# merijn-23/magr-ray-tracer

Hardware: AMD Instinct MI355X
Metric: Mrays/sec + extend-kernel HBM GB/s, sponza 1080p 256spp (higher is better)
Workload: dtype f32

## Files before the change

### include/rt355.h

```cpp
#ifndef RT355_H
#define RT355_H
#include "rt355_types.h"

#ifdef __cplusplus
extern "C" {
#endif

#define RT_OK            0
#define RT_E_INVALID    (-1)
#define RT_E_DEVICE     (-2)
#define RT_E_NOMEM      (-3)
#define RT_E_UNSUPPORTED (-4)

#define RT_SHADING_SIMPLE       0
#define RT_SHADING_NEE          1
#define RT_SAMPLING_HEMISPHERE  0
#define RT_SAMPLING_COSINE      1
#define RT_ACCEL_BVH2           0
#define RT_ACCEL_BVH4           1

typedef struct RtCtx RtCtx;

typedef struct RtConfig {
    int32_t width, height;
    int32_t y0, y1;
    int32_t max_bounces;
    int32_t shading, sampling, accel;
    int32_t russian_roulette;
    int32_t filter_fireflies;
    int32_t device;
    int32_t extend_variant;
    int32_t profile;
    int32_t shade_blocks_per_cu;
    int32_t persist_blocks_per_cu;
    int32_t builtins;
} RtConfig;

#define RT_BUILTINS_DEFAULT    0
#define RT_BUILTINS_IEEE       1
#define RT_BUILTINS_REFERENCE  2

typedef struct RtCounters {
    uint64_t extend_rays, extend_tlas_visits, extend_inst_visits, extend_node_visits, extend_prim_tests;
    uint64_t connect_rays, connect_tlas_visits, connect_inst_visits, connect_node_visits, connect_prim_tests;
    uint64_t primary_rays;
    uint64_t shadow_rays;
    uint64_t frames;
    uint64_t extend_node_issues, extend_leaf_issues, connect_node_issues, connect_leaf_issues;
    uint64_t extend_loop_node_events, extend_loop_leaf_events, connect_loop_node_events, connect_loop_leaf_events;
} RtCounters;

typedef struct RtStageTimes {
    double  generate_ms, extend_ms, shade_ms, compact_ms, connect_ms, accumulate_ms;
    int64_t generate_launches, extend_launches, shade_launches, compact_launches, connect_launches, accumulate_launches;
} RtStageTimes;

typedef struct RtKernelInfo {
    int32_t layout;
    int32_t persist, persist4;
    int32_t stack_entries;
    int32_t persist_grid, persist_grid_connect, shade_grid;
    int32_t n_blas;
} RtKernelInfo;

const char* rt_last_error(void);
int rt_device_count(void);
int rt_kernel_info(RtCtx* ctx, RtKernelInfo* out);
int rt_builtins(RtCtx* ctx);
int rt_top_levels(RtCtx* ctx, int32_t* extend, int32_t* connect);
typedef struct RtTraversalFacts {
    int32_t accel, extend_variant, persist_blocks_per_cu;
    int32_t layout;
    int32_t singleBlas;
    int32_t tlasDepth;
    int32_t nInterior, nQuads;
    int32_t stackEntries;
    int32_t sharedMemPerBlock;
    int32_t xcdFirst;
} RtTraversalFacts;
#define RT_TUNE_FIELDS 11
typedef struct RtTraversalPlan {
    int32_t trav;
    int32_t spillCap;
    int32_t coherent;
    int32_t topAuto;
    int32_t tuneBlocks, connectBlocks;
    int32_t tune[RT_TUNE_FIELDS], tuneConnect[RT_TUNE_FIELDS], tune4[RT_TUNE_FIELDS];
} RtTraversalPlan;
int rt_debug_traversal_plan(const RtTraversalFacts* facts, RtTraversalPlan* out);
int rt_debug_traversal_facts(RtCtx* ctx, RtTraversalFacts* out);
int rt_shade_footprint(RtCtx* ctx, int32_t* ldsBytes, int32_t* traversalBeside);
int rt_shade_tables(RtCtx* ctx, int32_t* capacityRows, int32_t* staged);

int rt_create(const RtConfig* cfg, RtCtx** out);
int rt_destroy(RtCtx* ctx);

int rt_upload_scene(RtCtx* ctx,
                    const RtPrimitive* prims, int32_t nPrims,
                    const RtMaterial* mats, int32_t nMats,
                    const RtFloat4* textures, int32_t nTexels,
                    const uint32_t* lights, int32_t nLights,
                    const void* bvhNodes, int32_t nNodes,
                    const uint32_t* primIdx, int32_t nIdx,
                    const RtTLASNode* tlas, int32_t nTlas,
                    const RtBVHInstance* blas, int32_t nBlas);

int rt_upload_scene_bvh2(RtCtx* ctx,
                         const RtPrimitive* prims, int32_t nPrims, const RtMaterial* mats, int32_t nMats,
                         const RtFloat4* textures, int32_t nTexels, const uint32_t* lights, int32_t nLights,
                         const RtBVHNode2* bvhNodes, int32_t nNodes, const uint32_t* primIdx, int32_t nIdx,
                         const RtTLASNode* tlas, int32_t nTlas, const RtBVHInstance* blas, int32_t nBlas);

int rt_validate_scene(int32_t accel,
                      const RtPrimitive* prims, int32_t nPrims, const RtMaterial* mats, int32_t nMats,
                      const RtFloat4* textures, int32_t nTexels, const uint32_t* lights, int32_t nLights,
                      const void* bvhNodes, int32_t nNodes, const uint32_t* primIdx, int32_t nIdx,
                      const RtTLASNode* tlas, int32_t nTlas, const RtBVHInstance* blas, int32_t nBlas);

int rt_share_scene(RtCtx* ctx, RtCtx* from);

int rt_build_bvh2(int32_t device, const RtBuildOptions* opts, const RtPrimitive* prims, int32_t nPrims, int32_t first, int32_t count,
                  uint32_t nodeBase, uint32_t idxBase, RtBVHNode2* nodes, int32_t nodeCap, int32_t* nNodes, uint32_t* primIdx,
                  RtBuildStats* stats);
int rt_build_bvh2_sah(int32_t device, const RtPrimitive* prims, int32_t nPrims, int32_t first, int32_t count, uint32_t nodeBase,
                      uint32_t idxBase, RtBVHNode2* nodes, int32_t nodeCap, int32_t* nNodes, uint32_t* primIdx, RtBuildStats* stats);
int rt_debug_sah_phases(float* out);
int rt_build_bvh2_sbvh(int32_t device, float alpha, const RtPrimitive* prims, int32_t nPrims, int32_t first, int32_t count,
                       uint32_t nodeBase, uint32_t idxBase, RtBVHNode2* nodes, int32_t nodeCap, int32_t* nNodes, uint32_t* primIdx,
                       int32_t idxCap, int32_t* nIdx, RtSbvhStats* stats);
int rt_debug_sbvh_phases(float* out);
int rt_build_bvh4(int32_t device, const RtBVHNode2* nodes2, int32_t nNodes, int32_t nIdx, const uint32_t* roots, int32_t nRoots,
                  RtBVHNode4* out4, RtBvh4Stats* stats);

typedef struct RtUpdateStats {
    double  gpu_ms;
    int32_t prims, nodes;
    int32_t tlas_nodes, tlas_depth;
    int32_t reconfigured;
    int32_t reserved[3];
} RtUpdateStats;
int rt_update_scene(RtCtx* ctx, const RtPrimitive* prims, int32_t first, int32_t count, const RtBVHInstance* blas, int32_t nBlas,
                    RtUpdateStats* stats);
#define RT_REBUILD_SAH   0
#define RT_REBUILD_LBVH  1
#define RT_REBUILD_SBVH  2
#define RT_REBUILD_REFIT 3
typedef struct RtRebuildStats {
    double  gpu_ms;
    double  wall_ms;
    double  stage_ms, build_ms, derive_ms, tlas_ms, commit_ms;
    int32_t prims, blas_built;
    int32_t nodes, n_idx;
    int32_t max_depth;
    int32_t tlas_nodes, tlas_depth;
    int32_t reconfigured;
    int32_t spatial_splits, prims_clipped;
} RtRebuildStats;
int rt_rebuild_scene(RtCtx* ctx, const RtPrimitive* prims, int32_t first, int32_t count, const RtBVHInstance* blas, int32_t nBlas,
                     int32_t builder, const RtBuildOptions* opts, RtRebuildStats* stats);
#define RT_REBUILD_KEEP  4
#define RT_REBUILD_REFIT_RANGE 5
int rt_rebuild_ranges(RtCtx* ctx, const RtPrimitive* prims, int32_t first, int32_t count, const RtBVHInstance* blas, int32_t nBlas,
                      const int32_t* plan, int32_t nRanges,
                      const RtBuildOptions* opts, RtRebuildStats* stats);
int rt_scene_blas_blocks(RtCtx* ctx, int32_t* n, int32_t* primFirst, int32_t* primCount, int32_t* nodes, int32_t* idxSlots, int32_t* compact, int32_t cap);
int rt_rebuild_ranges_check(int32_t nPrims, const int32_t* rangeFirst, const int32_t* rangeCount, const int32_t* compact, int32_t nBound,
                            const int32_t* plan, int32_t nRanges, int32_t first, int32_t count, const RtBuildOptions* opts);
typedef struct RtSceneShape {
    int32_t nRanges;
    const int32_t* rangeCount;
    int32_t nBlas;
    const int32_t* instRange;
    const RtBVHInstance* blas;
} RtSceneShape;
int rt_resize_scene(RtCtx* ctx, const void* prims, int32_t nPrims, const RtSceneShape* shape, int32_t builder, const RtBuildOptions* opts,
// ... 178 lines not shown
```

### magr_ray_tracer_amd/_lib.py

```python
import ctypes as C
import os

import numpy as np

_PKG = os.path.dirname(os.path.abspath(__file__))

f4 = np.dtype((np.float32, 4))
Ray = np.dtype([("O", f4), ("D", f4), ("rD", f4), ("N", f4), ("I", f4), ("intensity", f4), ("t", "<f4"),
                ("primIdx", "<i4"), ("bounces", "<i4"), ("pixelIdx", "<i4"), ("inside", "u1"), ("lastSpecular", "u1"),
                ("_pad0", "u1", 2), ("u", "<f4"), ("v", "<f4"), ("_pad1", "<u4")], align=False)
ShadowRay = np.dtype([("I", f4), ("L", f4), ("Nl", f4), ("intensity", f4), ("BRDF", f4), ("lightIdx", "<i4"),
                      ("pixelIdx", "<i4"), ("dotNL", "<f4"), ("dist", "<f4")])
Material = np.dtype([("color", f4), ("absorption", f4), ("specular", "<f4"), ("n1", "<f4"), ("n2", "<f4"),
                     ("isDielectric", "u1"), ("_pad0", "u1", 3), ("texIdx", "<i4"), ("texW", "<i4"), ("texH", "<i4"),
                     ("isLight", "u1"), ("_pad1", "u1", 3), ("emittance", f4)])
Primitive = np.dtype([("v0", f4), ("v1", f4), ("v2", f4), ("N", f4), ("centroid", f4), ("uv0", "<f4", 2), ("uv1", "<f4", 2),
                      ("uv2", "<f4", 2), ("_padt", "<f4", 2), ("objType", "<i4"), ("matIdx", "<i4"), ("area", "<f4"),
                      ("_pad", "<u4")])
Camera = np.dtype([("type", "<i4"), ("fov", "<f4"), ("aperture", "<f4"), ("focalLength", "<f4"), ("forward", f4),
                   ("right", f4), ("up", f4), ("origin", f4), ("horizontal", f4), ("vertical", f4), ("topLeft", f4)])
Settings = np.dtype([("numPrimitives", "<i4"), ("numLights", "<i4"), ("tracerType", "<i4"), ("frames", "<i4"),
                     ("antiAliasing", "<i4"), ("numInRays", "<i4"), ("numOutRays", "<i4"), ("shadowRays", "<i4"),
                     ("renderBVH", "<i4"), ("focalLength", "<f4")])
BVHNode2 = np.dtype([("aabbMin", f4), ("aabbMax", f4), ("first", "<u4"), ("count", "<u4"), ("_pad", "<u4", 2)])
# ... 20 lines not shown
SbvhStats = np.dtype([(n, "<i4") for n in ("nodes", "leaves", "n_idx", "depth", "spatial_splits", "prims_clipped", "forced_leaves", "levels")] +
                     [("sah_cost", "<f4"), ("device_ms", "<f4"), ("wall_ms", "<f4"), ("peak_refs", "<i4")])
Bvh4Stats = np.dtype([(n, "<i4") for n in ("live_nodes", "levels", "stack_need", "largest_leaf")] + [("device_ms", "<f4"), ("wall_ms", "<f4")])
Hit = np.dtype([("t", "<f4"), ("primIdx", "<i4"), ("u", "<f4"), ("v", "<f4")])
RayBatch = np.dtype([("origin", "<u8"), ("dir", "<u8"), ("originStride", "<i8"), ("dirStride", "<i8"), ("tmax", "<u8"), ("n", "<i8")])
TraceOut = np.dtype([("hit", "<u8"), ("point", "<u8"), ("normal", "<u8"), ("occluded", "<u8")])
TRACE_CLOSEST, TRACE_ANY = 0, 1
REALLYFAR = np.float32(1e30)
KernelInfo = np.dtype([(n, "<i4") for n in ("layout", "persist", "persist4", "stack_entries", "persist_grid", "persist_grid_connect",
                                             "shade_grid", "n_blas")])
TUNE_FIELDS = ("chunk", "refill", "inner", "leafK", "fixedChunks", "flat", "xcdRays", "xcdFirst", "thin", "topLevels", "topBase")
TraversalFacts = np.dtype([(n, "<i4") for n in ("accel", "extend_variant", "persist_blocks_per_cu", "layout", "singleBlas", "tlasDepth", "nInterior",
                                                 "nQuads", "stackEntries", "sharedMemPerBlock", "xcdFirst")])
TraversalPlan = np.dtype([(n, "<i4") for n in ("trav", "spillCap", "coherent", "topAuto", "tuneBlocks", "connectBlocks")] +
                         [(n, "<i4", len(TUNE_FIELDS)) for n in ("tune", "tuneConnect", "tune4")])
TRAV_NESTED, TRAV_BVH2, TRAV_TLAS, TRAV_TLAS_SPILL, TRAV_BVH4, TRAV_BVH4_TLAS, TRAV_BVH4_TLAS_SPILL = range(7)
assert TraversalFacts.itemsize == 44 and TraversalPlan.itemsize == 156

_SIZES = {"Ray": (Ray, 128), "ShadowRay": (ShadowRay, 96), "Material": (Material, 80), "Primitive": (Primitive, 128),
          "Camera": (Camera, 128), "Settings": (Settings, 40), "BVHNode2": (BVHNode2, 48), "BVHNode4": (BVHNode4, 160),
          "BVHInstance": (BVHInstance, 68), "TLASNode": (TLASNode, 48), "BuildOptions": (BuildOptions, 16), "BuildStats": (BuildStats, 32), "SbvhStats": (SbvhStats, 48), "Bvh4Stats": (Bvh4Stats, 24), "ShadowRecord": (ShadowRecord, 48), "Config": (Config, 64),
          "Hit": (Hit, 16), "RayBatch": (RayBatch, 48), "TraceOut": (TraceOut, 32)}
for _n, (_d, _s) in _SIZES.items():
    assert _d.itemsize == _s, (_n, _d.itemsize, _s)

SHADING_SIMPLE, SHADING_NEE = 0, 1
SAMPLING_HEMISPHERE, SAMPLING_COSINE = 0, 1
ACCEL_BVH2, ACCEL_BVH4 = 0, 1
PRIM_SPHERE, PRIM_PLANE, PRIM_TRIANGLE = 0, 1, 2
MATH_EXP, MATH_SIN, MATH_COS, MATH_ACOS, MATH_ATAN, MATH_F2I, MATH_ATAN2, MATH_SPHERE_TEXEL, MATH_NORMALIZE4, MATH_LENGTH4 = range(10)
MATH_WORDS = {MATH_EXP: (1, 1), MATH_SIN: (1, 1), MATH_COS: (1, 1), MATH_ACOS: (1, 1), MATH_ATAN: (1, 1), MATH_F2I: (1, 1),
              MATH_ATAN2: (2, 1), MATH_SPHERE_TEXEL: (6, 2), MATH_NORMALIZE4: (4, 4), MATH_LENGTH4: (4, 1)}
MATH_SWEEP_BLOCK_BITS = 20
MAX_BOUNCES = 7
BUILTINS_DEFAULT, BUILTINS_IEEE, BUILTINS_REFERENCE = 0, 1, 2
BUILTINS = {None: BUILTINS_DEFAULT, "ieee": BUILTINS_IEEE, "reference": BUILTINS_REFERENCE}


def builtins_value(name):
    try:
        return BUILTINS[name]
    except (KeyError, TypeError):
        raise ValueError(f"builtins must be None, 'ieee' or 'reference', not {name!r}") from None


RT_OK, RT_E_INVALID, RT_E_DEVICE, RT_E_NOMEM, RT_E_UNSUPPORTED = 0, -1, -2, -3, -4
SCENE_ARRAYS = {"prims": 0, "bvh": 1, "tlas": 2, "instances": 3, "pairs": 4, "triRecs": 5, "shadeRecs": 6, "lightRecs": 7,
                "tlasPairs": 8, "tlasPairsP": 9, "instRecs": 10}
SCENE_ARRAYS_BVH4 = {"quads": 11, "rootEntry": 12, "bvh2Kept": 13}
SCENE_ARRAYS_RESIZE = {"lights": 14}
SCENE_ARRAYS_MATERIALS = {"materials": 15, "textures": 16}
MaterialUpdate = np.dtype([("mats", "<u8"), ("nMats", "<i4"), ("_pad0", "<i4"), ("texels", "<u8"), ("texFirst", "<i4"), ("texCount", "<i4"),
                           ("nTexels", "<i4"), ("_pad1", "<i4"), ("primMat", "<u8"), ("primFirst", "<i4"), ("primCount", "<i4")])
assert MaterialUpdate.itemsize == 56
MaterialStats = np.dtype([("gpu_ms", "<f8"), ("wall_ms", "<f8")] +
                         [(n, "<i4") for n in ("mats", "texels", "prims", "lights", "tables_staged_changed", "atlas_reallocated")] +
                         [("reserved", "<i4", 2)])
assert MaterialStats.itemsize == 48
SceneShape = np.dtype([("nRanges", "<i4"), ("_pad0", "<i4"), ("rangeCount", "<u8"), ("nBlas", "<i4"), ("_pad1", "<i4"), ("instRange", "<u8"),
                       ("blas", "<u8")])
assert SceneShape.itemsize == 40
Geometry = np.dtype([("first", "<i4"), ("count", "<i4"), ("prims", "<u8"), ("positions", "<u8"), ("positionStride", "<i8"), ("nVertices", "<i8"),
                     ("indices", "<u8")])
assert Geometry.itemsize == 48
UpdateStats = np.dtype([("gpu_ms", "<f8"), ("prims", "<i4"), ("nodes", "<i4"), ("tlas_nodes", "<i4"), ("tlas_depth", "<i4"),
                        ("reconfigured", "<i4"), ("reserved", "<i4", 3)])
assert UpdateStats.itemsize == 40
REBUILD_SAH, REBUILD_LBVH, REBUILD_SBVH = 0, 1, 2
REBUILD_REFIT = 3
REBUILD_KEEP = 4
REBUILD_REFIT_RANGE = 5
RANGES_INFO_FIELDS = ("built", "kept", "refit", "pairs_derived", "pairs_relocated", "slots_derived", "slots_relocated", "nodes_numbered", "leaves_refit")
RangesInfo = np.dtype([(n, "<i4") for n in RANGES_INFO_FIELDS] + [("reserved", "<i4", 3)])
assert RangesInfo.itemsize == 48
RefitInfo = np.dtype([(n, "<i4") for n in ("path", "live_quads", "changed_nodes", "stack_need")])
assert RefitInfo.itemsize == 16
REFIT_NONE, REFIT_IN_PLACE, REFIT_RECOLLAPSED, REFIT_FORCED = 0, 1, 2, 3
RebuildStats = np.dtype([(n, "<f8") for n in ("gpu_ms", "wall_ms", "stage_ms", "build_ms", "derive_ms", "tlas_ms", "commit_ms")] +
                        [(n, "<i4") for n in ("prims", "blas_built", "nodes", "n_idx", "max_depth", "tlas_nodes", "tlas_depth", "reconfigured")] +
                        [("spatial_splits", "<i4"), ("prims_clipped", "<i4")])
assert RebuildStats.itemsize == 96

DEVICE_SYMBOLS = [
    "rt_last_error", "rt_device_count", "rt_kernel_info", "rt_builtins", "rt_top_levels", "rt_shade_footprint", "rt_shade_tables", "rt_create", "rt_destroy", "rt_upload_scene", "rt_share_scene", "rt_set_seeds", "rt_seed_default",
    "rt_get_seeds", "rt_bind_accum", "rt_accum_device_ptr", "rt_stream", "rt_reset", "rt_render", "rt_synchronize", "rt_focus",
    "rt_read_accum", "rt_write_accum", "rt_postproc", "rt_read_counters", "rt_reset_counters", "rt_read_stage_times", "rt_reset_stage_times", "rt_set_profile",
    "rt_stage_begin_frame", "rt_stage_generate", "rt_stage_extend", "rt_stage_shade", "rt_stage_connect",
    "rt_debug_get_rays", "rt_debug_set_rays", "rt_debug_get_shadow", "rt_debug_enable_steps", "rt_debug_get_steps", "rt_debug_math",
    "rt_debug_math_sweep", "rt_debug_math_mode", "rt_debug_math_sweep_mode", "rt_validate_scene", "rt_build_bvh2", "rt_build_bvh2_sah", "rt_debug_sah_phases", "rt_build_bvh2_sbvh", "rt_debug_sbvh_phases", "rt_update_scene", "rt_group_update_scene", "rt_debug_get_scene_array",
    "rt_rebuild_scene", "rt_group_rebuild_scene", "rt_blas_ranges", "rt_debug_rebuild_allocations", "rt_refit_info",
    "rt_build_bvh4", "rt_upload_scene_bvh2", "rt_group_upload_scene_bvh2",
    "rt_group_create", "rt_group_destroy", "rt_group_lanes", "rt_group_concurrency", "rt_group_stream_class", "rt_group_class_concurrency", "rt_group_lane", "rt_group_frames", "rt_group_upload_scene", "rt_group_share_scene",
    "rt_group_seed", "rt_group_reset", "rt_group_render", "rt_group_synchronize", "rt_group_sum", "rt_group_read_accum", "rt_group_focus",
    "rt_group_postproc", "rt_trace", "rt_trace_window", "rt_resize_scene", "rt_group_resize_scene", "rt_resize_check",
    "rt_update_materials", "rt_group_update_materials", "rt_materials_check",
    "rt_rebuild_ranges", "rt_group_rebuild_ranges", "rt_scene_blas_blocks", "rt_rebuild_ranges_check", "rt_blas_blocks",
    "rt_debug_traversal_plan", "rt_debug_traversal_facts", "rt_ranges_info", "rt_debug_derive_pairs", "rt_debug_relocate_pairs",
    "rt_update_geometry", "rt_rebuild_geometry", "rt_rebuild_geometry_ranges", "rt_group_update_geometry", "rt_group_rebuild_geometry",
    "rt_group_rebuild_geometry_ranges", "rt_geometry_check"]
HOST_SYMBOLS = [
    "rth_last_error", "rth_scene_create", "rth_scene_destroy", "rth_add_material", "rth_add_texture", "rth_load_texture", "rth_add_sphere",
    "rth_add_plane", "rth_add_triangle", "rth_add_quad", "rth_add_triangles", "rth_build_blas", "rth_build_bvh4",
    "rth_build_tlas", "rth_bvh4_from_nodes", "rth_set_instance_transform", "rth_primitives", "rth_materials", "rth_textures", "rth_lights",
    "rth_bvh2_nodes", "rth_bvh4_nodes", "rth_prim_idx", "rth_tlas_nodes", "rth_blas_nodes", "rth_bvh_stats", "rth_camera",
    "rth_renderer_create", "rth_renderer_destroy", "rth_renderer_init", "rth_renderer_set_camera", "rth_renderer_tick",
    "rth_renderer_read", "rth_renderer_camera", "rth_seed_stream", "rth_load_model", "rth_save_png",
    "rth_set_build_threads", "rth_renderer_save_frame", "rth_renderer_camera_move", "rth_renderer_camera_mouse", "rth_renderer_camera_zoom", "rth_renderer_frames", "rth_renderer_set_lanes", "rth_renderer_set_builtins", "rth_renderer_builtins",
    "rth_build_blas_lbvh", "rth_build_bvh2_lbvh", "rth_lbvh_stats", "rth_set_primitives", "rth_refit",
    "rth_build_blas_sah_gpu", "rth_build_bvh2_sah", "rth_build_blas_sbvh_gpu", "rth_build_bvh2_sbvh", "rth_rebuild", "rth_blas_ranges",
    "rth_build_bvh4_gpu", "rth_build_bvh4_levels", "rth_bvh4_refit", "rth_refit_bvh4", "rth_add_instance", "rth_light_list",
    "rth_set_materials", "rth_set_texels", "rth_set_prim_materials", "rth_rebuild_ranges", "rth_swap_instances", "rth_set_vertices"]

_dev = None
_host = None


class NativeLibraryMissing(RuntimeError):
    pass


def _load(name, local=False):
    path = os.path.join(_PKG, name)
    if not os.path.exists(path):
        raise NativeLibraryMissing(
            f"{path} is missing: build it with `python -m magr_ray_tracer_amd.build` (hipcc, gfx950). "
            "The hot path has no Python/CPU fallback.")
    return C.CDLL(path, mode=C.RTLD_LOCAL if local else C.RTLD_GLOBAL)


_variants = {}


def device_lib(variant=None):
    global _dev
    if variant:
        if variant not in _variants:
            keep, _dev = _dev, None
            try:
                _variants[variant] = _bind_device(_load(f"librt355_{variant}.so", local=True))
            finally:
                _dev = keep
        return _variants[variant]
    if _dev is None:
        _dev = _bind_device(_load("librt355.so"))
    return _dev


def _bind_device(lib):
    if True:
        vp, i32, i64 = C.c_void_p, C.c_int32, C.c_int64
        lib.rt_last_error.restype = C.c_char_p
        lib.rt_create.argtypes = [vp, C.POINTER(vp)]
        lib.rt_kernel_info.argtypes = [vp, vp]
        lib.rt_builtins.argtypes = [vp]
        lib.rt_top_levels.argtypes = [vp, C.POINTER(i32), C.POINTER(i32)]
        lib.rt_debug_traversal_plan.argtypes = [vp, vp]
        lib.rt_debug_traversal_facts.argtypes = [vp, vp]
        lib.rt_shade_footprint.argtypes = [vp, C.POINTER(i32), C.POINTER(i32)]
        lib.rt_shade_tables.argtypes = [vp, C.POINTER(i32), C.POINTER(i32)]
        lib.rt_destroy.argtypes = [vp]
        lib.rt_upload_scene.argtypes = [vp, vp, i32, vp, i32, vp, i32, vp, i32, vp, i32, vp, i32, vp, i32, vp, i32]
        lib.rt_upload_scene_bvh2.argtypes = lib.rt_upload_scene.argtypes
        lib.rt_group_upload_scene_bvh2.argtypes = lib.rt_upload_scene.argtypes
        lib.rt_build_bvh4.argtypes = [i32, vp, i32, i32, vp, i32, vp, vp]
        lib.rt_share_scene.argtypes = [vp, vp]
        lib.rt_set_seeds.argtypes = [vp, vp, i64]
        lib.rt_seed_default.argtypes = [vp]
        lib.rt_get_seeds.argtypes = [vp, vp, i64]
        lib.rt_bind_accum.argtypes = [vp, vp]
        lib.rt_accum_device_ptr.argtypes = [vp]
        lib.rt_accum_device_ptr.restype = vp
        lib.rt_stream.argtypes = [vp]
        lib.rt_stream.restype = vp
        lib.rt_reset.argtypes = [vp]
        lib.rt_render.argtypes = [vp, vp, vp, i32]
        lib.rt_synchronize.argtypes = [vp]
        lib.rt_focus.argtypes = [vp, i32, i32, vp, C.POINTER(C.c_float)]
        lib.rt_read_accum.argtypes = [vp, vp]
        lib.rt_read_counters.argtypes = [vp, vp]
        lib.rt_write_accum.argtypes = [vp, vp]
        lib.rt_postproc.argtypes = [vp, i32, C.c_float, C.c_float, C.c_float, vp, vp]
        lib.rt_reset_counters.argtypes = [vp]
        lib.rt_read_stage_times.argtypes = [vp, vp]
        lib.rt_reset_stage_times.argtypes = [vp]
        lib.rt_set_profile.argtypes = [vp, i32]
        lib.rt_stage_begin_frame.argtypes = [vp]
        lib.rt_stage_generate.argtypes = [vp, vp, vp]
        lib.rt_stage_extend.argtypes = [vp, i32, i32]
        lib.rt_stage_shade.argtypes = [vp, i32]
        lib.rt_stage_connect.argtypes = [vp, i32, i32]
        lib.rt_debug_get_rays.argtypes = [vp, i32, vp, i32, C.POINTER(i32)]
        lib.rt_debug_set_rays.argtypes = [vp, i32, vp, i32]
        lib.rt_trace.argtypes = [vp, i32, vp, vp]
        lib.rt_trace_window.argtypes = [vp]
        lib.rt_trace_window.restype = i64
        lib.rt_debug_get_shadow.argtypes = [vp, i32, i32, vp, i32, C.POINTER(i32)]
        lib.rt_debug_get_steps.argtypes = [vp, vp, i32, C.POINTER(i32)]
        lib.rt_debug_enable_steps.argtypes = [vp, i32]
        lib.rt_debug_math.argtypes = [i32, vp, vp, i64]
        lib.rt_debug_math_sweep.argtypes = [i32, i32, i32, vp]
        lib.rt_debug_math_mode.argtypes = [i32, i32, vp, vp, i64]
        lib.rt_debug_math_sweep_mode.argtypes = [i32, i32, i32, i32, vp]
        lib.rt_validate_scene.argtypes = [i32, vp, i32, vp, i32, vp, i32, vp, i32, vp, i32, vp, i32, vp, i32, vp, i32]
        lib.rt_build_bvh2.argtypes = [i32, vp, vp, i32, i32, i32, C.c_uint32, C.c_uint32, vp, i32, C.POINTER(i32), vp, vp]
        lib.rt_build_bvh2_sah.argtypes = [i32, vp, i32, i32, i32, C.c_uint32, C.c_uint32, vp, i32, C.POINTER(i32), vp, vp]
        lib.rt_debug_sah_phases.argtypes = [vp]
        lib.rt_build_bvh2_sbvh.argtypes = [i32, C.c_float, vp, i32, i32, i32, C.c_uint32, C.c_uint32, vp, i32, C.POINTER(i32), vp, i32, C.POINTER(i32), vp]
        lib.rt_debug_sbvh_phases.argtypes = [vp]
        lib.rt_update_scene.argtypes = [vp, vp, i32, i32, vp, i32, vp]
        lib.rt_group_update_scene.argtypes = [vp, vp, i32, i32, vp, i32, vp]
        lib.rt_debug_get_scene_array.argtypes = [vp, i32, vp, i64, C.POINTER(i64)]
        lib.rt_rebuild_scene.argtypes = [vp, vp, i32, i32, vp, i32, i32, vp, vp]
        lib.rt_group_rebuild_scene.argtypes = [vp, vp, i32, i32, vp, i32, i32, vp, vp]
        lib.rt_debug_rebuild_allocations.argtypes = [vp, vp]
        lib.rt_rebuild_ranges.argtypes = [vp, vp, i32, i32, vp, i32, vp, i32, vp, vp]
        lib.rt_group_rebuild_ranges.argtypes = [vp, vp, i32, i32, vp, i32, vp, i32, vp, vp]
        lib.rt_scene_blas_blocks.argtypes = [vp, vp, vp, vp, vp, vp, vp, i32]
        lib.rt_rebuild_ranges_check.argtypes = [i32, vp, vp, vp, i32, vp, i32, i32, i32, vp]
        lib.rt_blas_blocks.argtypes = [vp, i32, vp, i32, i32, vp, i32, vp, vp, vp, vp, vp, vp, i32]
        lib.rt_update_geometry.argtypes = [vp, vp, vp, i32, vp]
        lib.rt_group_update_geometry.argtypes = [vp, vp, vp, i32, vp]
        lib.rt_rebuild_geometry.argtypes = [vp, vp, vp, i32, i32, vp, vp]
        lib.rt_group_rebuild_geometry.argtypes = [vp, vp, vp, i32, i32, vp, vp]
        lib.rt_rebuild_geometry_ranges.argtypes = [vp, vp, vp, i32, vp, i32, vp, vp]
        lib.rt_group_rebuild_geometry_ranges.argtypes = [vp, vp, vp, i32, vp, i32, vp, vp]
        lib.rt_geometry_check.argtypes = [vp, i32, vp]
        lib.rt_resize_scene.argtypes = [vp, vp, i32, vp, i32, vp, vp]
        lib.rt_group_resize_scene.argtypes = [vp, vp, i32, vp, i32, vp, vp]
        lib.rt_resize_check.argtypes = [i32, vp, i32, vp]
        lib.rt_update_materials.argtypes = [vp, vp, vp]
        lib.rt_group_update_materials.argtypes = [vp, vp, vp]
        lib.rt_materials_check.argtypes = [vp, i32, i32]
        lib.rt_refit_info.argtypes = [vp, vp]
        lib.rt_ranges_info.argtypes = [vp, vp]
        lib.rt_debug_derive_pairs.argtypes = [vp, i32, vp, i32, vp, vp, i32, vp, C.POINTER(i32)]
        lib.rt_debug_relocate_pairs.argtypes = [vp, i32, C.c_uint32, C.c_uint32, vp]
        lib.rt_blas_ranges.argtypes = [vp, i32, vp, i32, i32, vp, i32, vp, vp]
        lib.rt_group_create.argtypes = [vp, i32, C.POINTER(vp)]
        lib.rt_group_destroy.argtypes = [vp]
        lib.rt_group_lanes.argtypes = [vp]
        lib.rt_group_concurrency.argtypes = [vp]
        lib.rt_group_stream_class.argtypes = [vp]
# ... 107 lines not shown
```

### magr_ray_tracer_amd/csrc/ctx.h

```cpp
#pragma once
#include <algorithm>
#include <memory>
#include <vector>
#include "rt355_dev.h"
#include "scene_dev.h"

struct RtCtx {
    RtConfig cfg{};
    hipStream_t stream = nullptr;
    hipStream_t home = nullptr;
    bool queued = true;
    rt355dev::DevScene sc{};
    rt355dev::DevQueues q{};
    rt355dev::DevVariant var{};
    int nPix = 0, firstPixel = 0, gridMax = 0;
    int cuCount = 0; size_t ldsPerBlock = 0, ldsPerCU = 0;
    bool sceneLoaded = false, ownAccum = true;
    std::shared_ptr<scenedev::SceneBag> scene;
    uint64_t sceneGen = 0;
    scenedev::SceneFacts facts;
    std::vector<void*> queueAllocs;
    float* dFocus = nullptr;
    RtRay* dRayIO = nullptr;
    uint64_t frames = 0, primaryRays = 0;
    struct Ev { hipEvent_t a, b; int stage; };
    std::vector<Ev> evPool; size_t evUsed = 0;
    RtStageTimes times{};
    int trav = 0;
    int coherent = 1;
    uint32_t* dSpill = nullptr; size_t spillWords = 0;
    int xcdFirst = -1;
    int spillCap = 0;
    bool cursorUsed[2 * (RT_MAX_BOUNCES + 2)] = {};
    bool shadeRun[RT_MAX_BOUNCES + 1] = {};
    bool generated = false;
    int persistGrid = 0, persistGridConnect = 0;
    rt355dev::PersistTune tune{}, tuneConnect{}, tune4{};
    int tuneBlocks = 0, connectBlocks = 0;
    float4* dPostF = nullptr; uchar4* dPostB = nullptr;
    int32_t* dSteps = nullptr;
    struct TraceView { rt355dev::DevQueues q{}; bool ready = false; std::vector<void*> words; float4* rays[3] = {}; size_t cap = 0; } tv;
    int shadeTile = rt355dev::kTile;
    int shadeGrid = 1024;
    void (*kGenerate)(rt355dev::DevQueues, RtCamera, int, int) = nullptr;
    void (*kShade)(rt355dev::DevScene, rt355dev::DevQueues, rt355dev::DevVariant, int) = nullptr;
    void (*kFocus)(rt355dev::DevScene, RtCamera, int, int, int, int, float*) = nullptr;
};

static inline dim3 grid_for(int n) { return dim3((unsigned)std::max(1, (n + rt355dev::kBlock - 1) / rt355dev::kBlock)); }
__attribute__((visibility("hidden"))) void ctx_free(RtCtx* ctx);
__attribute__((visibility("hidden"))) int postproc(RtCtx* ctx, const float4* accum, int32_t frames, float vignette, float gamma, float chromatic,
                                                    RtFloat4* outF32, uint8_t* outRGBA8);
```

### magr_ray_tracer_amd/csrc/rt355.hip

```cpp
#include <hip/hip_runtime.h>
#include <hip/hip_ext.h>
#include <algorithm>
#include <cstdio>
#include <cmath>
#include <cstdlib>
#include <cstring>
#include <memory>
#include <atomic>
#include <string>
#include <vector>
#include "../../include/rt355.h"
#include "rt355_kernels.h"
#include "ctx.h"
#include "geometry_common.h"

using namespace rt355dev;
using namespace scenedev;

static_assert(kColumnLanes == kBlock && kTopLevelsMax == kTopMaxLevels && sizeof(float4) * 4 == 64, "trav_common.h computes with the kernels' sizes");
static thread_local std::string g_err;
int rt355_set_error(int code, const char* msg) { g_err = msg; return code; }

template <bool REFB> static void choose_builtin_kernels_of(RtCtx* ctx)
{
    const bool nee = ctx->cfg.shading == RT_SHADING_NEE, small = ctx->shadeTile == 256;
    ctx->kGenerate = k_generate<REFB>;
    ctx->kShade = nee ? (small ? k_shade<true, 256, REFB> : k_shade<true, kTile, REFB>) : (small ? k_shade<false, 256, REFB> : k_shade<false, kTile, REFB>);
    ctx->kFocus = ctx->cfg.accel == RT_ACCEL_BVH4 ? k_focus<RT_ACCEL_BVH4, REFB> : k_focus<RT_ACCEL_BVH2, REFB>;
}
static void choose_builtin_kernels(RtCtx* ctx)
{
    if (ctx->cfg.builtins == RT_BUILTINS_REFERENCE) choose_builtin_kernels_of<true>(ctx);
    else choose_builtin_kernels_of<false>(ctx);
}
enum { ST_GENERATE, ST_EXTEND, ST_SHADE, ST_COMPACT, ST_CONNECT, ST_ACCUM };

extern "C" const char* rt_last_error(void) { return g_err.c_str(); }
extern "C" int rt_device_count(void) { int n = 0; if (hipGetDeviceCount(&n) != hipSuccess) return 0; return n; }
static int sync_scene_config(RtCtx* ctx);
extern "C" int rt_builtins(RtCtx* ctx)
{
    if (!ctx) return fail(RT_E_INVALID, "rt_builtins: null context");
    return ctx->cfg.builtins;
}
extern "C" int rt_kernel_info(RtCtx* ctx, RtKernelInfo* out)
{
    if (!ctx || !out) return fail(RT_E_INVALID, "rt_kernel_info: null argument");
    if (!ctx->sceneLoaded) return fail(RT_E_INVALID, "rt_kernel_info: no scene uploaded");
    if (const int rc = sync_scene_config(ctx)) return rc;
    const int persist = ctx->trav <= TRAV_TLAS_SPILL ? ctx->trav : 0;
    const int persist4 = ctx->trav == TRAV_BVH4 ? 1 : (ctx->trav == TRAV_BVH4_TLAS ? 2 : (ctx->trav == TRAV_BVH4_TLAS_SPILL ? 3 : 0));
    *out = RtKernelInfo{ ctx->facts.layout, persist, persist4, spill_trav(ctx->trav) ? ctx->spillCap : ctx->facts.stackEntries, ctx->persistGrid, ctx->persistGridConnect,
                         ctx->shadeGrid, ctx->sc.nBlas };
    return RT_OK;
}

extern "C" int rt_top_levels(RtCtx* ctx, int32_t* extend, int32_t* connect)
{
    if (!ctx || !extend || !connect) return fail(RT_E_INVALID, "rt_top_levels: null argument");
    if (!ctx->sceneLoaded) return fail(RT_E_INVALID, "rt_top_levels: no scene uploaded");
    if (const int rc = sync_scene_config(ctx)) return rc;
    *extend = ctx->tune.topLevels; *connect = ctx->tuneConnect.topLevels;
    return RT_OK;
}

static int beside_shade(const RtCtx* c, int stage, int topLevels, int* perCU, int* shadeLds);
extern "C" int rt_shade_footprint(RtCtx* ctx, int32_t* ldsBytes, int32_t* traversalBeside)
{
    if (!ctx || !ldsBytes || !traversalBeside) return fail(RT_E_INVALID, "rt_shade_footprint: null argument");
    if (!ctx->sceneLoaded) return fail(RT_E_INVALID, "rt_shade_footprint: no scene uploaded");
    if (const int rc = sync_scene_config(ctx)) return rc;
    *ldsBytes = 0; *traversalBeside = 0;
    if (!persistent(ctx->trav)) {
        hipFuncAttributes a{};
        HIPCHK(hipFuncGetAttributes(&a, (const void*)ctx->kShade));
        *ldsBytes = (int32_t)a.sharedSizeBytes;
        return RT_OK;
    }
    int lds = 0, beside = 0;
    if (const int rc = beside_shade(ctx, ST_EXTEND, 0, &beside, &lds)) return rc;
    *ldsBytes = lds; *traversalBeside = beside;
    return RT_OK;
}

extern "C" int rt_shade_tables(RtCtx* ctx, int32_t* capacityRows, int32_t* staged)
{
    if (!ctx || !capacityRows || !staged) return fail(RT_E_INVALID, "rt_shade_tables: null argument");
    if (!ctx->sceneLoaded) return fail(RT_E_INVALID, "rt_shade_tables: no scene uploaded");
    if (const int rc = sync_scene_config(ctx)) return rc;
    *capacityRows = kShadeTableRows;
    *staged = ctx->var.shadeTables != 0 && shade_tables_fit(ctx->sc.nLights, ctx->sc.nMats);
    return RT_OK;
}

static void free_bag(std::vector<void*>& bag) { for (void* p : bag) (void)hipFree(p); bag.clear(); }

static void scene_release(RtCtx* ctx)
{
    if (!ctx->scene) return;
    auto& h = ctx->scene->holders;
    h.erase(std::remove(h.begin(), h.end(), ctx), h.end());
    ctx->scene.reset();
}
static void scene_hold(RtCtx* ctx, const std::shared_ptr<SceneBag>& bag)
{
    scene_release(ctx);
    ctx->scene = bag;
    bag->holders.push_back(ctx);
}
int SceneBag::wait_holders() const
{
    for (const RtCtx* h : holders) {
        HIPCHK(hipStreamSynchronize(h->stream));
        if (h->home != h->stream) HIPCHK(hipStreamSynchronize(h->home));
    }
    return RT_OK;
}

static int tlas_lds_entries(const RtCtx* c) { return tlas_lds_entries(c->trav, c->spillCap, c->facts.stackEntries, c->facts.tlasDepth); }
static size_t tlas_stack_bytes(const RtCtx* c) { return tlas_column_bytes(tlas_lds_entries(c)); }

using PersistKernel = void (*)(DevScene, DevQueues, int, int, int, PersistTune);
using NestedKernel = void (*)(DevScene, DevQueues, int, int);
struct TraceLaunch {
    PersistKernel persist = nullptr;
    NestedKernel nested = nullptr;
    dim3 grid;
    size_t lds = 0;
    PersistTune tune{};
};
static TraceLaunch trace_launch(const RtCtx* c, int stage, int bounce, bool steps, int rays, int topLevels = -1 )
{
    TraceLaunch L;
    L.grid = grid_for(rays);
    L.lds = stack_bytes(c->facts.stackEntries);
    const bool connect = stage == ST_CONNECT;
    const bool bvh4 = c->cfg.accel == RT_ACCEL_BVH4, l1 = c->facts.layout == 1;
    bool top = false;
    switch (c->trav) {
    case TRAV_NESTED:
        if (connect) L.nested = bvh4 ? (l1 ? k_connect<RT_ACCEL_BVH4, 1> : k_connect<RT_ACCEL_BVH4, 0>) : (l1 ? k_connect<RT_ACCEL_BVH2, 1> : k_connect<RT_ACCEL_BVH2, 0>);
        else L.nested = bvh4 ? (l1 ? k_extend<RT_ACCEL_BVH4, 1> : k_extend<RT_ACCEL_BVH4, 0>) : (l1 ? k_extend<RT_ACCEL_BVH2, 1> : k_extend<RT_ACCEL_BVH2, 0>);
        break;
    case TRAV_BVH2:
        L.tune = connect ? c->tuneConnect : c->tune;
        if (topLevels >= 0) L.tune.topLevels = topLevels;
        if (connect) { top = L.tune.topLevels > 0; L.persist = top ? k_trace_persist<true, false, false, true> : k_trace_persist<true>; L.grid = dim3(c->persistGridConnect); }
        else if (bounce > 0 || c->cfg.extend_variant == 3) {
            top = L.tune.topLevels > 0;
            if (top) L.persist = steps ? k_trace_persist<false, false, true, true> : k_trace_persist<false, false, false, true>;
            else L.persist = steps ? k_trace_persist<false, false, true> : k_trace_persist<false>;
            L.grid = dim3(c->persistGrid);
        }
        else if (c->cfg.extend_variant == 5) L.nested = k_extend<RT_ACCEL_BVH2, 1>;
        else L.persist = c->coherent ? k_trace_persist<false, true> : (steps ? k_trace_persist<false, false, true> : k_trace_persist<false>);
        if (top) { L.tune.topBase = c->facts.stackEntries * kBlock; L.lds += top_bytes(L.tune.topLevels); }
        break;
    case TRAV_BVH4:
        L.tune = connect ? c->tuneConnect : c->tune4;
        L.persist = connect ? k_trace_persist4<true> : k_trace_persist4<false>;
        if (connect || bounce > 0) L.grid = dim3(connect ? c->persistGridConnect : c->persistGrid);
        break;
    case TRAV_TLAS:
    case TRAV_TLAS_SPILL: {
        const bool spill = c->trav == TRAV_TLAS_SPILL;
        L.lds = tlas_stack_bytes(c);
        if (connect) {
            L.tune = c->tuneConnect;
            L.persist = spill ? k_trace_persist_tlas<true, false, true> : k_trace_persist_tlas<true>;
            L.grid = dim3(c->persistGridConnect);
            break;
        }
        L.tune = c->tune;
        if (bounce > 0 || spill) L.grid = dim3(c->persistGrid);
        const bool coh = c->coherent && (bounce == 0 || c->coherent == 2) && (c->tune.flat || !spill);
        if (steps) L.persist = spill ? k_trace_persist_tlas<false, true, true> : k_trace_persist_tlas<false, true>;
        else if (coh) L.persist = spill ? k_trace_persist_tlas<false, false, true, true> : k_trace_persist_tlas<false, false, false, true>;
        else L.persist = spill ? k_trace_persist_tlas<false, false, true> : k_trace_persist_tlas<false>;
        break;
    }
    case TRAV_BVH4_TLAS:
    case TRAV_BVH4_TLAS_SPILL: {
        const bool spill = c->trav == TRAV_BVH4_TLAS_SPILL;
        L.lds = tlas_stack_bytes(c);
        if (connect) {
            L.tune = c->tuneConnect;
            L.persist = spill ? k_trace_persist4_tlas<true, false, true> : k_trace_persist4_tlas<true>;
            L.grid = dim3(c->persistGridConnect);
            break;
        }
        L.tune = c->tune4;
        if (bounce > 0 || spill) L.grid = dim3(c->persistGrid);
        if (steps) L.persist = spill ? k_trace_persist4_tlas<false, true, true> : k_trace_persist4_tlas<false, true>;
        else L.persist = spill ? k_trace_persist4_tlas<false, false, true> : k_trace_persist4_tlas<false>;
        break;
    }
    }
    return L;
}

static int persist_query(const RtCtx* c, int stage, int topLevels, int* perCU)
{
    const TraceLaunch L = trace_launch(c, stage, stage == ST_CONNECT ? 0 : 1, false, c->nPix, topLevels);
    HIPCHK(hipOccupancyMaxActiveBlocksPerMultiprocessor(perCU, L.persist, kBlock, L.lds));
    return RT_OK;
}
static int persist_blocks(const RtCtx* c, int stage, int perCU)
{
    const bool connect = stage == ST_CONNECT;
    const int fit = std::max(1, perCU);
    int g = std::max(1, std::min(perCU, connect ? kAdmitAnySgpr : kAdmit96Sgpr));
    if (c->cfg.persist_blocks_per_cu > 0) g = std::min(g, std::min(c->cfg.persist_blocks_per_cu, fit));
    if (c->tuneBlocks > 0) g = std::min(c->tuneBlocks, fit);
    if (connect && c->connectBlocks > 0) g = std::min(c->connectBlocks, fit);
    return g;
}

static constexpr size_t kLdsBlock = 1280;
static int beside_shade(const RtCtx* c, int stage, int topLevels, int* perCU, int* shadeLds)
{
    const TraceLaunch L = trace_launch(c, stage, stage == ST_CONNECT ? 0 : 1, false, c->nPix, topLevels);
    hipFuncAttributes shade{}, trav{};
    HIPCHK(hipFuncGetAttributes(&shade, (const void*)c->kShade));
    HIPCHK(hipFuncGetAttributes(&trav, (const void*)L.persist));
    auto alloc = [](int regs) { return std::max(8, (regs + 7) / 8 * 8); };
    const size_t ldsCU = std::max(c->ldsPerCU, c->ldsPerBlock);
    auto blocks = [](size_t bytes) { return (bytes + kLdsBlock - 1) / kLdsBlock * kLdsBlock; };
    const size_t travLds = blocks(trav.sharedSizeBytes + L.lds), shadeLdsCU = blocks(shade.sharedSizeBytes);
    const int shadeWaves = std::max(1, c->shadeTile / kBlock);
    const int byLds = ldsCU > shadeLdsCU && travLds > 0 ? (int)((ldsCU - shadeLdsCU) / travLds) : 0;
    const int byVgpr = (512 - shadeWaves * alloc(shade.numRegs)) / alloc(trav.numRegs);
    const int bySlots = 8 - shadeWaves;
    *perCU = std::max(0, std::min(std::min(byLds, byVgpr), std::min(bySlots, stage == ST_CONNECT ? kAdmitAnySgpr : kAdmit96Sgpr)));
    *shadeLds = (int)shade.sharedSizeBytes;
    return RT_OK;
}

static constexpr size_t kEvRing = 4096;
static void ev_account(RtCtx* c, RtCtx::Ev& e)
{
    float ms = 0;
    if (hipEventElapsedTime(&ms, e.a, e.b) != hipSuccess) { (void)hipEventSynchronize(e.b); (void)hipEventElapsedTime(&ms, e.a, e.b); }
    switch (e.stage) {
    case ST_GENERATE: c->times.generate_ms += ms; c->times.generate_launches++; break;
// ... 84 lines not shown
        choose_builtin_kernels(ctx);
        HIPCHK(hipOccupancyMaxActiveBlocksPerMultiprocessor(&perCU, ctx->kShade, ctx->shadeTile, 0));
        perCU = std::min(perCU, kAdmitAnySgpr);
        ctx->shadeGrid = ctx->cuCount * std::max(1, perCU);
        if (c.shade_blocks_per_cu > 0 && c.shade_blocks_per_cu <= 16) ctx->shadeGrid = ctx->cuCount * c.shade_blocks_per_cu;
        if (knobs.perCU) ctx->shadeGrid = ctx->cuCount * knobs.perCU;
    }
    hipError_t e = hipStreamCreateWithFlags(&ctx->home, hipStreamNonBlocking);
    if (e != hipSuccess) return fail(RT_E_DEVICE, "hipStreamCreate failed: %s", hipGetErrorString(e));
    ctx->stream = ctx->home;
    DevQueues& q = ctx->q;
    const size_t n = (size_t)ctx->nPix, nS = n * (size_t)c.max_bounces;
    int rc = RT_OK;
    auto& bag = ctx->queueAllocs;
#define QA(field, count) if (rc == RT_OK) rc = dalloc(bag, &q.field, count)
    const size_t nTiles = (n + kBlock - 1) / kBlock;
    for (int k = 0; k < 2; k++) { QA(O[k], n); QA(D[k], n); QA(inten[k], n); QA(meta[k], n); QA(tile[k], nTiles + 2); QA(super[k], nTiles / 64 + 2); QA(supAcc[k], nTiles / 64 + 2); }
    QA(hit, n);
    QA(sA, nS); QA(sB, nS); QA(sC, nS);
    QA(nRays, RT_MAX_BOUNCES + 2); QA(nShadow, RT_MAX_BOUNCES + 2); QA(cursor, kCursorWords); QA(shadeTicket, (size_t)(RT_MAX_BOUNCES + 1) * kTicketClasses * kTicketStride); QA(fault, 1);
    QA(seeds, n); QA(accum, (size_t)c.width * c.height);
    if (rc == RT_OK) rc = dalloc(bag, &ctx->dSteps, n);
    q.steps = nullptr;
    QA(ctrExtend, (size_t)ctx->gridMax * kCtrCols); QA(ctrConnect, (size_t)ctx->gridMax * kCtrCols);
#undef QA
    if (rc == RT_OK) rc = dalloc(bag, &ctx->dFocus, 1);
    if (rc != RT_OK) return rc;
    q.nPix = ctx->nPix; q.firstPixel = ctx->firstPixel; q.width = c.width; q.height = c.height;
    (void)hipMemsetAsync(q.accum, 0, sizeof(float4) * (size_t)c.width * c.height, ctx->stream);
    (void)hipMemsetAsync(q.nRays, 0, sizeof(int32_t) * (RT_MAX_BOUNCES + 2), ctx->stream);
    (void)hipMemsetAsync(q.nShadow, 0, sizeof(int32_t) * (RT_MAX_BOUNCES + 2), ctx->stream);
    (void)hipMemsetAsync(q.cursor, 0, sizeof(int32_t) * kCursorWords, ctx->stream);
    (void)hipMemsetAsync(q.shadeTicket, 0, sizeof(int32_t) * (size_t)(RT_MAX_BOUNCES + 1) * kTicketClasses * kTicketStride, ctx->stream);
    (void)hipMemsetAsync(q.fault, 0, sizeof(int32_t), ctx->stream);
    (void)hipMemsetAsync(q.ctrExtend, 0, sizeof(unsigned long long) * (size_t)ctx->gridMax * kCtrCols, ctx->stream);
    (void)hipMemsetAsync(q.ctrConnect, 0, sizeof(unsigned long long) * (size_t)ctx->gridMax * kCtrCols, ctx->stream);
    for (int k = 0; k < 2; k++) {
        (void)hipMemsetAsync(q.tile[k], 0, sizeof(unsigned long long) * (nTiles + 2), ctx->stream);
        (void)hipMemsetAsync(q.super[k], 0, sizeof(unsigned long long) * (nTiles / 64 + 2), ctx->stream);
        (void)hipMemsetAsync(q.supAcc[k], 0, sizeof(unsigned long long) * (nTiles / 64 + 2), ctx->stream);
    }
    (void)hipMemsetAsync(q.hit, 0, sizeof(float4) * n, ctx->stream);
    HIPCHK(hipStreamSynchronize(ctx->stream));
    rc = rt_seed_default(ctx);
    if (rc != RT_OK) return rc;
    ev_init(ctx);
    *out = guard.release();
    return RT_OK;
}

void ctx_free(RtCtx* ctx)
{
    if (!ctx) return;
    (void)hipSetDevice(ctx->cfg.device);
    if (ctx->stream) (void)hipStreamSynchronize(ctx->stream);
    scene_release(ctx); free_bag(ctx->queueAllocs);
    if (ctx->dRayIO) (void)hipFree(ctx->dRayIO);
    free_bag(ctx->tv.words);
    for (float4* p : ctx->tv.rays) if (p) (void)hipFree(p);
    if (ctx->dSpill) (void)hipFree(ctx->dSpill);
    if (ctx->dPostF) (void)hipFree(ctx->dPostF);
    if (ctx->dPostB) (void)hipFree(ctx->dPostB);
    for (auto& e : ctx->evPool) { if (e.a) (void)hipEventDestroy(e.a); if (e.b) (void)hipEventDestroy(e.b); }
    if (ctx->home) (void)hipStreamDestroy(ctx->home);
    delete ctx;
}
extern "C" int rt_destroy(RtCtx* ctx)
{
    ctx_free(ctx);
    return RT_OK;
}

static TravFacts traversal_facts(const RtCtx* ctx)
{
    const SceneFacts& s = ctx->facts;
    return TravFacts{ ctx->cfg.accel, ctx->cfg.extend_variant, ctx->cfg.persist_blocks_per_cu, s.layout, s.singleBlas, s.tlasDepth, s.nInterior, s.nQuads, s.stackEntries,
                      (int)ctx->ldsPerBlock, ctx->xcdFirst };
}
static void adopt_plan(RtCtx* ctx, const TravPlan& p)
{
    ctx->trav = p.trav; ctx->spillCap = p.spillCap; ctx->coherent = p.coherent;
    ctx->tune = p.tune; ctx->tuneConnect = p.tuneConnect; ctx->tune4 = p.tune4;
    ctx->tuneBlocks = p.tuneBlocks; ctx->connectBlocks = p.connectBlocks;
}
static int fit_top_tables(RtCtx* ctx, bool topAuto)
{
    for (PersistTune* t : { &ctx->tune, &ctx->tuneConnect }) if (stack_bytes(ctx->facts.stackEntries) + top_bytes(t->topLevels) > ctx->ldsPerBlock) t->topLevels = 0;
    if (topAuto) for (int stage : { ST_EXTEND, ST_CONNECT }) {
        PersistTune& t = stage == ST_CONNECT ? ctx->tuneConnect : ctx->tune;
        int q = 0, lv = t.topLevels, beside = 0, shadeLds = 0;
        const bool shared = ctx->cfg.persist_blocks_per_cu > 0;
        if (const int rc = persist_query(ctx, stage, 0, &q)) return rc;
        const int base = persist_blocks(ctx, stage, q);
        if (shared) { if (const int rc = beside_shade(ctx, stage, 0, &beside, &shadeLds)) return rc; }
        for (; lv > 0; lv--) {
            if (const int rc = persist_query(ctx, stage, lv, &q)) return rc;
            if (persist_blocks(ctx, stage, q) != base) continue;
            if (!shared) break;
            int fit = 0;
            if (const int rc = beside_shade(ctx, stage, lv, &fit, &shadeLds)) return rc;
            if (fit >= beside) break;
        }
        t.topLevels = lv;
    }
    return RT_OK;
}
static int size_persistent_grids(RtCtx* ctx)
{
    int perCU = 0;
    if (const int rc = persist_query(ctx, ST_EXTEND, -1, &perCU)) return rc;
    int perCUc = perCU;
    if (bvh4_tlas_trav(ctx->trav) || ctx->tuneConnect.topLevels > 0) { if (const int rc = persist_query(ctx, ST_CONNECT, -1, &perCUc)) return rc; }
    ctx->persistGrid = std::min(ctx->gridMax, persist_blocks(ctx, ST_EXTEND, perCU) * ctx->cuCount);
    ctx->persistGridConnect = std::min(ctx->gridMax, persist_blocks(ctx, ST_CONNECT, perCUc) * ctx->cuCount);
    return RT_OK;
}
static int bind_spill_columns(RtCtx* ctx)
{
    ctx->q.spill = nullptr; ctx->q.spillStride = 0; ctx->q.stackCap = 0;
    ctx->q.tlasLdsEntries = tlas_trav(ctx->trav) ? (uint32_t)tlas_lds_entries(ctx) : 0u;
    if (!spill_trav(ctx->trav)) return RT_OK;
    const size_t stride = (size_t)std::max(ctx->persistGrid, ctx->persistGridConnect) * kBlock;
    const size_t words = stride * (size_t)(tlas_stack_entries(ctx->facts.stackEntries, ctx->facts.tlasDepth) - ctx->spillCap);
    if (words > ctx->spillWords) {
        if (ctx->dSpill) (void)hipFree(ctx->dSpill);
        ctx->dSpill = nullptr; ctx->spillWords = 0;
        if (hipMalloc((void**)&ctx->dSpill, words * sizeof(uint32_t)) != hipSuccess) return fail(RT_E_NOMEM, "hipMalloc of the spill stacks (%zu bytes) failed", words * sizeof(uint32_t));
        ctx->spillWords = words;
    }
    ctx->q.spill = ctx->dSpill; ctx->q.spillStride = (uint32_t)stride; ctx->q.stackCap = (uint32_t)ctx->spillCap;
    return RT_OK;
}
static int configure_traversal(RtCtx* ctx)
{
    static std::atomic<int> serial{ 0 };
    if (ctx->xcdFirst < 0) ctx->xcdFirst = serial.fetch_add(1) & 7;
    const TravPlan plan = plan_traversal(traversal_facts(ctx), read_trav_knobs());
    adopt_plan(ctx, plan);
    if (persistent(ctx->trav)) {
        if (const int rc = fit_top_tables(ctx, plan.topAuto)) return rc;
        if (const int rc = size_persistent_grids(ctx)) return rc;
    } else ctx->persistGrid = ctx->persistGridConnect = 0;
    return bind_spill_columns(ctx);
}

static void frame_state_reset(RtCtx* ctx);
static int adopt_scene(RtCtx* ctx)
{
    const SceneBag& b = *ctx->scene;
    const SceneArrays& a = b.sc;
    if (ctx->sceneLoaded && ctx->sc.nPrims != a.nPrims) {
        const DevQueues& q = ctx->q;
        HIPCHK(hipMemsetAsync(q.nRays, 0, sizeof(int32_t) * (RT_MAX_BOUNCES + 2), ctx->stream));
        HIPCHK(hipMemsetAsync(q.nShadow, 0, sizeof(int32_t) * (RT_MAX_BOUNCES + 2), ctx->stream));
        HIPCHK(hipMemsetAsync(q.cursor, 0, sizeof(int32_t) * kCursorWords, ctx->stream));
        HIPCHK(hipMemsetAsync(q.shadeTicket, 0, sizeof(int32_t) * (size_t)(RT_MAX_BOUNCES + 1) * kTicketClasses * kTicketStride, ctx->stream));
        HIPCHK(hipMemsetAsync(q.hit, 0, sizeof(float4) * (size_t)ctx->nPix, ctx->stream));
        ctx->queued = true;
        frame_state_reset(ctx);
    }
    auto f4 = [](const RtFloat4* p) { return (const float4*)p; };
    ctx->sc = DevScene{ a.prims, a.mats, f4(a.tex), a.lights, a.bvh2, a.bvh4, a.primIdx, a.tlas, a.blas, f4(a.pairs), f4(a.triRecs), a.rootEntry, f4(a.shadeRecs),
                        f4(a.tlasPairs), f4(a.instRecs), a.tlasRoot, f4(a.tlasPairsP), a.tlasRootP, f4(a.lightRecs), f4(a.quads), a.nLights, a.nPrims, a.nBlas, a.nTex, a.nMats };
    ctx->facts = b.facts;
    const int rc = configure_traversal(ctx);
    if (rc == RT_OK) ctx->sceneGen = b.generation;
// ... 272 lines not shown
    return RT_OK;
}
extern "C" int rt_bind_accum(RtCtx* ctx, void* devicePtr)
{
    if (!ctx) return fail(RT_E_INVALID, "rt_bind_accum: null context");
    HIPCHK(hipSetDevice(ctx->cfg.device));
    HIPCHK(hipStreamSynchronize(ctx->stream));
    if (devicePtr) { ctx->q.accum = (float4*)devicePtr; ctx->ownAccum = false; }
    else if (!ctx->ownAccum) {
        float4* a = nullptr;
        int rc = dalloc(ctx->queueAllocs, &a, (size_t)ctx->cfg.width * ctx->cfg.height);
        if (rc != RT_OK) return rc;
        HIPCHK(hipMemset(a, 0, sizeof(float4) * (size_t)ctx->cfg.width * ctx->cfg.height));
        ctx->q.accum = a; ctx->ownAccum = true;
    }
    return RT_OK;
}
extern "C" void* rt_accum_device_ptr(RtCtx* ctx) { return ctx ? (void*)ctx->q.accum : nullptr; }
extern "C" void* rt_stream(RtCtx* ctx) { if (ctx) ctx->queued = true; return ctx ? (void*)ctx->stream : nullptr; }

extern "C" int rt_reset(RtCtx* ctx)
{
    if (!ctx) return fail(RT_E_INVALID, "rt_reset: null context");
    HIPCHK(hipSetDevice(ctx->cfg.device));
    ctx->queued = true;
    hipLaunchKernelGGL(k_reset, dim3((ctx->nPix + kBlock - 1) / kBlock), dim3(kBlock), 0, ctx->stream, ctx->q.accum, ctx->firstPixel, ctx->nPix);
    HIPCHK(hipGetLastError());
    return RT_OK;
}

static int need_scene(RtCtx* ctx, const char* who)
{
    if (!ctx) return fail(RT_E_INVALID, "%s: null context", who);
    if (!ctx->sceneLoaded) return fail(RT_E_INVALID, "%s: no scene uploaded", who);
    return sync_scene_config(ctx);
}

static void frame_state_reset(RtCtx* ctx)
{
    memset(ctx->cursorUsed, 0, sizeof ctx->cursorUsed);
    memset(ctx->shadeRun, 0, sizeof ctx->shadeRun);
    ctx->generated = false;
}
extern "C" int rt_stage_begin_frame(RtCtx* ctx)
{
    if (!ctx) return fail(RT_E_INVALID, "rt_stage_begin_frame: null context");
    ctx->queued = true;
    hipLaunchKernelGGL(k_begin_frame, dim3(1), dim3(256), 0, ctx->stream, ctx->q);
    HIPCHK(hipGetLastError());
    frame_state_reset(ctx);
    return RT_OK;
}
static int generate(RtCtx* ctx, const RtCamera* cam, const RtSettings* s, int beginFrame)
{
    if (beginFrame) frame_state_reset(ctx);
    ctx->queued = true;
    LAUNCH(ctx, ST_GENERATE, ctx->kGenerate, grid_for(ctx->nPix), 0, ctx->q, *cam, s ? s->antiAliasing : 1, beginFrame);
    HIPCHK(hipGetLastError());
    ctx->primaryRays += (uint64_t)ctx->nPix;
    ctx->generated = true;
    return RT_OK;
}
extern "C" int rt_stage_generate(RtCtx* ctx, const RtCamera* cam, const RtSettings* s)
{
    if (!ctx || !cam) return fail(RT_E_INVALID, "rt_stage_generate: null argument");
    return generate(ctx, cam, s, 0);
}
extern "C" int rt_stage_extend(RtCtx* ctx, int32_t bounce, int32_t renderBVH)
{
    int rc = need_scene(ctx, "rt_stage_extend"); if (rc) return rc;
    ctx->queued = true;
    if (bounce < 0 || bounce > ctx->cfg.max_bounces) return fail(RT_E_INVALID, "rt_stage_extend: bounce %d outside [0, %d]", bounce, ctx->cfg.max_bounces);
    if (persistent(ctx->trav)) {
        if (ctx->cursorUsed[bounce]) HIPCHK(hipMemsetAsync(ctx->q.cursor + bounce, 0, sizeof(int32_t), ctx->stream));
        ctx->cursorUsed[bounce] = true;
    }
    const bool wantSteps = renderBVH != 0 || ctx->q.steps != nullptr;
    const TraceLaunch L = trace_launch(ctx, ST_EXTEND, bounce, wantSteps, ctx->nPix);
    if (L.persist) LAUNCH(ctx, ST_EXTEND, L.persist, L.grid, L.lds, ctx->sc, ctx->q, bounce, bounce, renderBVH, L.tune);
    else LAUNCH(ctx, ST_EXTEND, L.nested, L.grid, L.lds, ctx->sc, ctx->q, bounce, renderBVH);
    HIPCHK(hipGetLastError());
    return RT_OK;
}
extern "C" int rt_stage_shade(RtCtx* ctx, int32_t bounce)
{
    int rc = need_scene(ctx, "rt_stage_shade"); if (rc) return rc;
    ctx->queued = true;
    if (bounce < 0 || bounce >= ctx->cfg.max_bounces) return fail(RT_E_INVALID, "rt_stage_shade: bounce %d outside [0, %d)", bounce, ctx->cfg.max_bounces);
    if (ctx->shadeRun[bounce] || (bounce > 0 && !ctx->shadeRun[bounce - 1]) || (bounce == 0 && !ctx->generated)) {
        const size_t nTiles = ((size_t)ctx->nPix + kBlock - 1) / kBlock;
        HIPCHK(hipMemsetAsync(ctx->q.tile[bounce & 1], 0, sizeof(unsigned long long) * (nTiles + 2), ctx->stream));
        HIPCHK(hipMemsetAsync(ctx->q.super[bounce & 1], 0, sizeof(unsigned long long) * (nTiles / 64 + 2), ctx->stream));
        HIPCHK(hipMemsetAsync(ctx->q.supAcc[bounce & 1], 0, sizeof(unsigned long long) * (nTiles / 64 + 2), ctx->stream));
        HIPCHK(hipMemsetAsync(ctx->q.shadeTicket + (size_t)bounce * kTicketClasses * kTicketStride, 0, sizeof(int32_t) * (size_t)kTicketClasses * kTicketStride, ctx->stream));
    }
    const int tileSz = ctx->shadeTile;
    const dim3 sg((unsigned)std::max(1, std::min(ctx->shadeGrid, (ctx->nPix + tileSz - 1) / tileSz)));
    LAUNCHB(ctx, ST_SHADE, ctx->kShade, sg, tileSz, 0, ctx->sc, ctx->q, ctx->var, bounce);
    ctx->shadeRun[bounce] = true;
    HIPCHK(hipGetLastError());
    return RT_OK;
}
extern "C" int rt_stage_connect(RtCtx* ctx, int32_t b0, int32_t b1)
{
    int rc = need_scene(ctx, "rt_stage_connect"); if (rc) return rc;
    ctx->queued = true;
    if (b0 < 0 || b1 < b0 || b1 >= ctx->cfg.max_bounces) return fail(RT_E_INVALID, "rt_stage_connect: bounce range [%d,%d] outside [0, %d)", b0, b1, ctx->cfg.max_bounces);
    if (persistent(ctx->trav)) {
        const int ci = (RT_MAX_BOUNCES + 2) + b0;
        if (ctx->cursorUsed[ci]) HIPCHK(hipMemsetAsync(ctx->q.cursor + ci, 0, sizeof(int32_t), ctx->stream));
        ctx->cursorUsed[ci] = true;
    }
    const TraceLaunch L = trace_launch(ctx, ST_CONNECT, b0, false, ctx->nPix * (b1 - b0 + 1));
    if (L.persist) LAUNCH(ctx, ST_CONNECT, L.persist, L.grid, L.lds, ctx->sc, ctx->q, b0, b1, 0, L.tune);
    else LAUNCH(ctx, ST_CONNECT, L.nested, L.grid, L.lds, ctx->sc, ctx->q, b0, b1);
    ev_begin(ctx, ST_ACCUM);
    for (int b = b0; b <= b1; b++)
        hipLaunchKernelGGL(k_accumulate, dim3(std::min(grid_for(ctx->nPix).x, 2048u)), dim3(kBlock), 0, ctx->stream, ctx->q, b);
    ev_end(ctx, ST_ACCUM);
    HIPCHK(hipGetLastError());
    return RT_OK;
}

static constexpr int64_t kTraceWindowMax = (int64_t)1 << 22;
static int64_t trace_window(const RtCtx* ctx)
{
    int64_t w = std::min<int64_t>((int64_t)ctx->gridMax * kBlock, kTraceWindowMax);
    if (const char* t = getenv("RT355_TRACE_WINDOW")) { const long long k = atoll(t); if (k > 0) w = std::min<int64_t>(w, k); }
    return w;
}
extern "C" int64_t rt_trace_window(RtCtx* ctx)
{
    if (!ctx) return fail(RT_E_INVALID, "rt_trace_window: null context");
    return trace_window(ctx);
}
static int device_pointer(const RtCtx* ctx, const char* who, const char* name, const void* p, int64_t bytes, int align, bool hostAllowed, bool* onDevice)
{
    if ((uintptr_t)p % (uintptr_t)align) return fail(RT_E_INVALID, "%s: %s (%p) is not aligned to %d bytes", who, name, p, align);
    hipPointerAttribute_t a{};
    const hipError_t e = hipPointerGetAttributes(&a, p);
    if (e != hipSuccess) (void)hipGetLastError();
    const bool device = e == hipSuccess && a.type == hipMemoryTypeDevice && a.device == ctx->cfg.device;
    const bool shared = e == hipSuccess && (a.type == hipMemoryTypeManaged || (a.type == hipMemoryTypeHost && a.devicePointer == p));
    const bool host = e != hipSuccess || a.type == hipMemoryTypeUnregistered || a.type == hipMemoryTypeHost;
    if (!device && !shared && !(hostAllowed && host))
        return fail(RT_E_INVALID, "%s: %s (%p) is not memory accessible from device %d (a host pointer? memory of another GPU?)", who, name, p, ctx->cfg.device);
    if (device) {
        hipDeviceptr_t base = nullptr; size_t size = 0;
        if (hipMemGetAddressRange(&base, &size, (hipDeviceptr_t)p) != hipSuccess) (void)hipGetLastError();
        else if ((const char*)p + bytes > (const char*)base + size)
            return fail(RT_E_INVALID, "%s: %s needs %lld bytes from %p, its allocation ends %lld bytes earlier", who, name, (long long)bytes, p,
                        (long long)(((const char*)p + bytes) - ((const char*)base + size)));
    }
    if (onDevice) *onDevice = device || shared;
    return RT_OK;
}
static int trace_pointer(const RtCtx* ctx, const char* name, const void* p, int64_t bytes, int align) { return device_pointer(ctx, "rt_trace", name, p, bytes, align, false); }
static int trace_view(RtCtx* ctx, size_t ownRays)
{
    RtCtx::TraceView& v = ctx->tv;
    if (!v.ready) {
        DevQueues q{};
        unsigned long long* ctr = nullptr;
        int rc = dalloc(v.words, &q.nRays, RT_MAX_BOUNCES + 2);
        if (rc == RT_OK) rc = dalloc(v.words, &q.nShadow, RT_MAX_BOUNCES + 2);
        if (rc == RT_OK) rc = dalloc(v.words, &q.cursor, kCursorWords);
        if (rc == RT_OK) rc = dalloc(v.words, &q.fault, 1);
        if (rc == RT_OK) rc = dalloc(v.words, &ctr, (size_t)ctx->gridMax * kCtrCols);
        if (rc != RT_OK) { free_bag(v.words); return rc; }
        HIPCHK(hipMemsetAsync(q.nRays, 0, sizeof(int32_t) * (RT_MAX_BOUNCES + 2), ctx->stream));
        HIPCHK(hipMemsetAsync(q.nShadow, 0, sizeof(int32_t) * (RT_MAX_BOUNCES + 2), ctx->stream));
        HIPCHK(hipMemsetAsync(q.cursor, 0, sizeof(int32_t) * kCursorWords, ctx->stream));
        HIPCHK(hipMemsetAsync(q.fault, 0, sizeof(int32_t), ctx->stream));
        HIPCHK(hipMemsetAsync(ctr, 0, sizeof(unsigned long long) * (size_t)ctx->gridMax * kCtrCols, ctx->stream));
        q.ctrExtend = q.ctrConnect = ctr;
        q.nPix = ctx->nPix; q.firstPixel = ctx->firstPixel; q.width = ctx->cfg.width; q.height = ctx->cfg.height;
        v.q = q; v.ready = true;
    }
    if (ownRays > v.cap) {
        HIPCHK(hipStreamSynchronize(ctx->stream));
        for (float4*& p : v.rays) { if (p) (void)hipFree(p); p = nullptr; }
        v.cap = 0;
        for (float4*& p : v.rays)
            if (hipMalloc((void**)&p, ownRays * sizeof(float4)) != hipSuccess) {
                (void)hipGetLastError();
                for (float4*& r : v.rays) { if (r) (void)hipFree(r); r = nullptr; }
                return fail(RT_E_NOMEM, "rt_trace: hipMalloc of the query's ray arrays (3 x %zu bytes) failed", ownRays * sizeof(float4));
            }
        v.cap = ownRays;
    }
    return RT_OK;
}
extern "C" int rt_trace(RtCtx* ctx, int32_t mode, const RtRayBatch* rays, const RtTraceOut* out)
{
    if (!ctx) return fail(RT_E_INVALID, "rt_trace: null ctx");
    if (!rays) return fail(RT_E_INVALID, "rt_trace: null rays");
    if (!out) return fail(RT_E_INVALID, "rt_trace: null out");
    int rc = need_scene(ctx, "rt_trace"); if (rc) return rc;
    if (mode != RT_TRACE_CLOSEST && mode != RT_TRACE_ANY) return fail(RT_E_INVALID, "rt_trace: mode %d is neither RT_TRACE_CLOSEST (0) nor RT_TRACE_ANY (1)", mode);
    const bool any = mode == RT_TRACE_ANY;
    const int64_t n = rays->n;
    if (n < 0) return fail(RT_E_INVALID, "rt_trace: rays->n = %lld is negative", (long long)n);
    if (rays->originStride < 12 || rays->originStride % 4) return fail(RT_E_INVALID, "rt_trace: rays->originStride = %lld must be >= 12 and a multiple of 4", (long long)rays->originStride);
    if (rays->dirStride < 12 || rays->dirStride % 4) return fail(RT_E_INVALID, "rt_trace: rays->dirStride = %lld must be >= 12 and a multiple of 4", (long long)rays->dirStride);
    if (any) {
        if (out->hit || out->point || out->normal) return fail(RT_E_INVALID, "rt_trace: out->%s is not produced by RT_TRACE_ANY", out->hit ? "hit" : (out->point ? "point" : "normal"));
    } else if (out->occluded) return fail(RT_E_INVALID, "rt_trace: out->occluded is not produced by RT_TRACE_CLOSEST");
    if (n == 0) return RT_OK;
    if (any ? !out->occluded : !out->hit) return fail(RT_E_INVALID, "rt_trace: out->%s is required by %s", any ? "occluded" : "hit", any ? "RT_TRACE_ANY" : "RT_TRACE_CLOSEST");
    if (!rays->origin) return fail(RT_E_INVALID, "rt_trace: null rays->origin");
    if (!rays->dir) return fail(RT_E_INVALID, "rt_trace: null rays->dir");
    HIPCHK(hipSetDevice(ctx->cfg.device));
    if ((rc = trace_pointer(ctx, "rays->origin", rays->origin, (n - 1) * rays->originStride + 12, 4))) return rc;
    if ((rc = trace_pointer(ctx, "rays->dir", rays->dir, (n - 1) * rays->dirStride + 12, 4))) return rc;
    if (rays->tmax) if ((rc = trace_pointer(ctx, "rays->tmax", rays->tmax, n * 4, 4))) return rc;
    if (out->hit) if ((rc = trace_pointer(ctx, "out->hit", out->hit, n * 16, 16))) return rc;
    if (out->point) if ((rc = trace_pointer(ctx, "out->point", out->point, n * 16, 16))) return rc;
    if (out->normal) if ((rc = trace_pointer(ctx, "out->normal", out->normal, n * 16, 16))) return rc;
    if (out->occluded) if ((rc = trace_pointer(ctx, "out->occluded", out->occluded, n, 1))) return rc;
    const bool vecO = rays->originStride == 16 && (uintptr_t)rays->origin % 16 == 0, vecD = rays->dirStride == 16 && (uintptr_t)rays->dir % 16 == 0;
    const bool inPlace = !any && vecO && vecD && !rays->tmax && !out->point && !out->normal;
    const int64_t window = trace_window(ctx);
    if ((rc = trace_view(ctx, inPlace ? 0 : (size_t)std::min(n, window)))) return rc;
    ctx->queued = true;
    DevQueues q = ctx->tv.q;
    q.spill = ctx->q.spill; q.spillStride = ctx->q.spillStride; q.stackCap = ctx->q.stackCap; q.tlasLdsEntries = ctx->q.tlasLdsEntries;
    for (int64_t off = 0; off < n; off += window) {
        const int m = (int)std::min(window, n - off);
        TraceIO io{ (const char*)rays->origin + off * rays->originStride, (const char*)rays->dir + off * rays->dirStride, rays->originStride, rays->dirStride,
                    rays->tmax ? rays->tmax + off : nullptr, out->hit ? (float4*)out->hit + off : nullptr, out->point ? (float4*)out->point + off : nullptr,
                    out->normal ? (float4*)out->normal + off : nullptr, out->occluded ? out->occluded + off : nullptr };
        float4* const* own = ctx->tv.rays;
        q.O[kTraceBounce & 1] = q.sA = inPlace ? (float4*)io.origin : own[0];
        q.D[kTraceBounce & 1] = q.sB = inPlace ? (float4*)io.dir : own[1];
        q.hit = q.sC = inPlace ? io.hit : own[2];
        hipLaunchKernelGGL(k_trace_arm, dim3(1), dim3(1), 0, ctx->stream, q, m, (int)any);
        if (!inPlace) hipLaunchKernelGGL(k_trace_load, grid_for(m), dim3(kBlock), 0, ctx->stream, q, io, m, (int)any, (int)vecO, (int)vecD);
        const TraceLaunch L = trace_launch(ctx, any ? ST_CONNECT : ST_EXTEND, kTraceBounce, false, m);
        if (L.persist) hipLaunchKernelGGL(L.persist, L.grid, dim3(kBlock), L.lds, ctx->stream, ctx->sc, q, kTraceBounce, kTraceBounce, 0, L.tune);
        else if (any) hipLaunchKernelGGL(L.nested, L.grid, dim3(kBlock), L.lds, ctx->stream, ctx->sc, q, kTraceBounce, kTraceBounce);
        else hipLaunchKernelGGL(L.nested, L.grid, dim3(kBlock), L.lds, ctx->stream, ctx->sc, q, kTraceBounce, 0);
        if (!inPlace) hipLaunchKernelGGL(k_trace_store, grid_for(m), dim3(kBlock), 0, ctx->stream, ctx->sc, q, io, m, (int)any);
        HIPCHK(hipGetLastError());
    }
    return RT_OK;
}

extern "C" int rt_render(RtCtx* ctx, const RtCamera* cam, const RtSettings* settings, int32_t frames)
{
    int rc = need_scene(ctx, "rt_render"); if (rc) return rc;
    if (!cam) return fail(RT_E_INVALID, "rt_render: null camera");
    if (frames <= 0) return fail(RT_E_INVALID, "rt_render: frames must be > 0");
    HIPCHK(hipSetDevice(ctx->cfg.device));
    const bool nee = ctx->cfg.shading == RT_SHADING_NEE, rr = ctx->cfg.russian_roulette != 0;
    const int renderBVH = settings ? settings->renderBVH : 0;
    for (int f = 0; f < frames; f++) {
        if ((rc = generate(ctx, cam, settings, 1))) return rc;
        for (int b = 0; b < ctx->cfg.max_bounces; b++) {
            if ((rc = rt_stage_extend(ctx, b, renderBVH))) return rc;
            if (renderBVH) break;
            if ((rc = rt_stage_shade(ctx, b))) return rc;
            if (!rr && nee) if ((rc = rt_stage_connect(ctx, b, b))) return rc;
        }
        if (rr && nee && !renderBVH) if ((rc = rt_stage_connect(ctx, 0, ctx->cfg.max_bounces - 1))) return rc;
        ctx->frames++;
    }
    return RT_OK;
}
static int check_fault(RtCtx* ctx)
{
    int32_t f = 0;
    HIPCHK(hipMemcpy(&f, ctx->q.fault, sizeof f, hipMemcpyDeviceToHost));
    if (f) {
        (void)hipMemset(ctx->q.fault, 0, sizeof f);
        return fail(RT_E_DEVICE, "device fault 0x%08x: a bounded wait of the ordered scan in k_shade expired (results of this render are invalid)", (unsigned)f);
    }
    return RT_OK;
}
extern "C" int rt_synchronize(RtCtx* ctx)
{
    if (!ctx) return fail(RT_E_INVALID, "rt_synchronize: null context");
    HIPCHK(hipSetDevice(ctx->cfg.device));
    HIPCHK(hipStreamSynchronize(ctx->stream));
    ev_collect(ctx);
    return check_fault(ctx);
}

extern "C" int rt_focus(RtCtx* ctx, int32_t x, int32_t y, const RtCamera* cam, float* t)
{
    int rc = need_scene(ctx, "rt_focus"); if (rc) return rc;
    if (!cam || !t) return fail(RT_E_INVALID, "rt_focus: null argument");
    HIPCHK(hipSetDevice(ctx->cfg.device));
    hipLaunchKernelGGL(ctx->kFocus, dim3(1), dim3(kBlock), stack_bytes(ctx->facts.stackEntries), ctx->stream, ctx->sc, *cam, x, y, ctx->cfg.width, ctx->cfg.height, ctx->dFocus);
    HIPCHK(hipGetLastError());
    HIPCHK(hipMemcpyAsync(t, ctx->dFocus, sizeof(float), hipMemcpyDeviceToHost, ctx->stream));
    HIPCHK(hipStreamSynchronize(ctx->stream));
    return RT_OK;
}

extern "C" int rt_read_accum(RtCtx* ctx, RtFloat4* out)
{
    if (!ctx || !out) return fail(RT_E_INVALID, "rt_read_accum: null argument");
    HIPCHK(hipSetDevice(ctx->cfg.device));
    HIPCHK(hipStreamSynchronize(ctx->stream));
    ev_collect(ctx);
    int rc = check_fault(ctx); if (rc) return rc;
    HIPCHK(hipMemcpy(out, ctx->q.accum, sizeof(float4) * (size_t)ctx->cfg.width * ctx->cfg.height, hipMemcpyDeviceToHost));
    return RT_OK;
}
extern "C" int rt_write_accum(RtCtx* ctx, const RtFloat4* in)
{
    if (!ctx || !in) return fail(RT_E_INVALID, "rt_write_accum: null argument");
    HIPCHK(hipSetDevice(ctx->cfg.device));
    HIPCHK(hipStreamSynchronize(ctx->stream));
    HIPCHK(hipMemcpy(ctx->q.accum, in, sizeof(float4) * (size_t)ctx->cfg.width * ctx->cfg.height, hipMemcpyHostToDevice));
    return RT_OK;
}
static int sum_table(RtCtx* ctx, const unsigned long long* dev, uint64_t out[kCtrCols])
{
    std::vector<unsigned long long> h((size_t)ctx->gridMax * kCtrCols);
    HIPCHK(hipMemcpy(h.data(), dev, h.size() * sizeof(unsigned long long), hipMemcpyDeviceToHost));
    for (int k = 0; k < kCtrCols; k++) out[k] = 0;
    for (size_t b = 0; b < (size_t)ctx->gridMax; b++) for (int k = 0; k < kCtrCols; k++) out[k] += h[b * kCtrCols + k];
    return RT_OK;
}
extern "C" int rt_read_counters(RtCtx* ctx, RtCounters* out)
{
    if (!ctx || !out) return fail(RT_E_INVALID, "rt_read_counters: null argument");
    HIPCHK(hipSetDevice(ctx->cfg.device));
    HIPCHK(hipStreamSynchronize(ctx->stream));
    ev_collect(ctx);
    uint64_t e[kCtrCols], c[kCtrCols];
    int rc = sum_table(ctx, ctx->q.ctrExtend, e); if (rc) return rc;
    rc = sum_table(ctx, ctx->q.ctrConnect, c); if (rc) return rc;
    memset(out, 0, sizeof *out);
    out->extend_rays = e[0]; out->extend_tlas_visits = e[1]; out->extend_inst_visits = e[2]; out->extend_node_visits = e[3]; out->extend_prim_tests = e[4];
    out->connect_rays = c[0]; out->connect_tlas_visits = c[1]; out->connect_inst_visits = c[2]; out->connect_node_visits = c[3]; out->connect_prim_tests = c[4];
    out->primary_rays = ctx->primaryRays; out->shadow_rays = c[0]; out->frames = ctx->frames;
    out->extend_node_issues = e[5]; out->extend_leaf_issues = e[6]; out->connect_node_issues = c[5]; out->connect_leaf_issues = c[6];
    out->extend_loop_node_events = e[7]; out->extend_loop_leaf_events = e[8]; out->connect_loop_node_events = c[7]; out->connect_loop_leaf_events = c[8];
    return RT_OK;
}
extern "C" int rt_reset_counters(RtCtx* ctx)
{
// ... 159 lines not shown
```

### magr_ray_tracer_amd/csrc/rt355_dev.h

```cpp
#pragma once
#include <hip/hip_runtime.h>
#include <stdint.h>
#include "../../include/rt355_types.h"
#include "trav_common.h"

namespace rt355dev {

#define RT_FORCEINLINE __device__ __forceinline__
static constexpr int   kBlock = 256;

struct DevScene {
    const RtPrimitive*   prims;
    const RtMaterial*    mats;
    const float4*        tex;
    const uint32_t*      lights;
    const RtBVHNode2*    bvh2;
    const RtBVHNode4*    bvh4;
    const uint32_t*      primIdx;
    const RtTLASNode*    tlas;
    const RtBVHInstance* blas;
    const float4*        pairs;
    const float4*        triRecs;
    const uint32_t*      rootEntry;
    const float4*        shadeRecs;
    const float4*        tlasPairs;
    const float4*        instRecs;
    uint32_t             tlasRoot;
    const float4*        tlasPairsP;
    uint32_t             tlasRootP;
    const float4*        lightRecs;
    const float4*        quads;
    int32_t nLights, nPrims, nBlas, nTex;
    int32_t nMats;
};
struct DevQueues {
    float4* O[2]; float4* D[2]; float4* inten[2]; uint2* meta[2];
    float4* hit;
    float4* sA; float4* sB; float4* sC;
    unsigned long long* tile[2];
    unsigned long long* super[2];
    unsigned long long* supAcc[2];
    int32_t* nRays;
    int32_t* nShadow;
    int32_t* fault;
    int32_t* cursor;
    int32_t* shadeTicket;
    uint32_t* seeds;
    float4* accum;
    int32_t* steps;
    unsigned long long* ctrExtend;
    unsigned long long* ctrConnect;
    uint32_t* spill;
    uint32_t spillStride, stackCap;
    uint32_t tlasLdsEntries;
    int32_t nPix, firstPixel, width, height;
};
static constexpr int kTicketClasses = 1, kTicketStride = 1024, kCursorWords = 2 * (RT_MAX_BOUNCES + 2);
struct DevVariant { int32_t shading, sampling, accel, rr, fireflies, maxBounces, shadeTables ; };
static constexpr int kCtrCols = 9;
static constexpr int kTile = 512;

}
```

### magr_ray_tracer_amd/csrc/rt355_kernels.h

```cpp
#pragma once
#include <hip/hip_runtime.h>
#include <stdint.h>
#include "../../include/rt355_types.h"
#include "rt355_dev.h"
#include "rt355_math.h"
#include "collapse_common.h"

namespace rt355dev {

using namespace refit;
using collapse::quad_min; using collapse::quad_max; using collapse::quad_entry;

static constexpr float kEps = RT_EPSILON;
static constexpr float kFar = RT_REALLYFAR;
static constexpr float kPi = 3.14159274101257f;
static constexpr float kInvPi = 0.31830987334251f;

static constexpr uint32_t kMetaBounceMask = 0xffu, kMetaInside = 0x100u, kMetaLastSpec = 0x200u;

RT_FORCEINLINE uint32_t rng_next(uint32_t& s) { s ^= s << 13; s ^= s >> 17; s ^= s << 5; return s; }
RT_FORCEINLINE float rnd_float(uint32_t& s) { return (float)rng_next(s) * 2.3283064365387e-10f; }
RT_FORCEINLINE float rnd_abs(uint32_t& s) { return fabsf(rnd_float(s)); }
RT_FORCEINLINE float4 rnd_float3(uint32_t& s) { float x = rnd_float(s), y = rnd_float(s), z = rnd_float(s); return mk4(x, y, z, 0.0f); }

// ... 345 lines not shown
RT_FORCEINLINE int traverse_instance(const DevScene& sc, TRay& r, uint32_t instIdx, uint32_t* stk, WorkCtr& wc)
{
    const float4* ir = sc.instRecs + (size_t)instIdx * 4;
    const float4 t0 = ir[0], t1 = ir[1], t2 = ir[2], t3 = ir[3];
    const float bx = r.ox, by = r.oy, bz = r.oz, bdx = r.dx, bdy = r.dy, bdz = r.dz, brx = r.rx, bry = r.ry, brz = r.rz;
    transform_ray(r, t0, t1, t2);
    wc.inst++;
    const uint32_t rootEnc = inst_root(t3), bvhIdx = inst_bvh(t3);
    int steps;
    if (ACCEL == RT_ACCEL_BVH4) steps = LAYOUT == 1 ? traverse_bvh4_packed<OCC>(sc, r, rootEnc, stk, wc) : traverse_bvh4<OCC>(sc, r, bvhIdx, stk, wc);
    else if (LAYOUT == 1) steps = traverse_bvh2_packed<OCC>(sc, r, rootEnc, stk, wc);
    else steps = traverse_bvh2<OCC>(sc, r, bvhIdx, stk, wc);
    r.ox = bx; r.oy = by; r.oz = bz; r.dx = bdx; r.dy = bdy; r.dz = bdz; r.rx = brx; r.ry = bry; r.rz = brz;
    return steps;
}

template <int ACCEL, int LAYOUT, bool OCC>
RT_FORCEINLINE int traverse_tlas(const DevScene& sc, TRay& r, uint32_t* stk, WorkCtr& wc)
{
    uint16_t tstack[RT_TLAS_STACK];
    uint32_t cur = sc.tlasRoot, sp = 0;
    int steps = 0;
    const float tLight = r.t;
    for (;;) {
        if (plain_leaf(cur)) {
            int value = traverse_instance<ACCEL, LAYOUT, OCC>(sc, r, plain_inst(cur), stk, wc);
            if (OCC && value == -1) return -1;
            steps += value;
            if (sp == 0) break;
            cur = tlas_unpack16(tstack[--sp]);
            continue;
        }
        wc.tlas++;
        const float4* p = sc.tlasPairs + (size_t)cur * 4;
        const float4 q0 = p[0], q1 = p[1], q2 = p[2], q3 = p[3];
        float d1 = slab(r, pair_min1(q0, q1, q2), pair_max1(q0, q1, q2));
        float d2 = slab(r, pair_min2(q0, q1, q2), pair_max2(q0, q1, q2));
        uint32_t c1 = pair_entry1(q3), c2 = pair_entry2(q3);
        if (d1 > d2) { float d = d1; d1 = d2; d2 = d; uint32_t c = c1; c1 = c2; c2 = c; }
        if (d1 >= tLight) {
            if (sp == 0) break;
            cur = tlas_unpack16(tstack[--sp]);
        } else {
            cur = c1;
            if (d2 < tLight) tstack[sp++] = tlas_pack16(c2);
        }
    }
    return steps;
}

RT_FORCEINLINE void flush_counters(unsigned long long* table, uint32_t rays, const WorkCtr& wc, uint32_t* red )
{
    uint32_t v[kCtrCols] = { rays, wc.tlas, wc.inst, wc.node, wc.prim, wc.nodeIss, wc.leafIss, wc.evNode, wc.evPrim };
#pragma unroll
    for (int k = 0; k < kCtrCols; k++)
#pragma unroll
        for (int off = 32; off > 0; off >>= 1) v[k] += __shfl_xor(v[k], off, 64);
    const int wave = threadIdx.x >> 6, lane = threadIdx.x & 63;
    __syncthreads();
    if (lane == 0) for (int k = 0; k < kCtrCols; k++) red[wave * kCtrCols + k] = v[k];
    __syncthreads();
    if (threadIdx.x < kCtrCols) {
        unsigned long long s = 0;
        for (int w = 0; w < kBlock / 64; w++) s += red[w * kCtrCols + threadIdx.x];
        table[(size_t)blockIdx.x * kCtrCols + threadIdx.x] += s;
    }
}

__global__ void k_reset(float4* accum, int32_t first, int32_t n)
{
    int i = blockIdx.x * blockDim.x + threadIdx.x;
    if (i < n) accum[first + i] = splat(0.0f);
}
RT_FORCEINLINE void begin_frame(const DevQueues& q)
{
    if (threadIdx.x == 0) { q.nRays[0] = q.nPix; q.nShadow[0] = 0; }
    if (threadIdx.x < kCursorWords) q.cursor[threadIdx.x] = 0;
    for (int k = threadIdx.x; k < (RT_MAX_BOUNCES + 1) * kTicketClasses; k += blockDim.x) q.shadeTicket[(size_t)k * kTicketStride] = 0;
}
__global__ void k_begin_frame(DevQueues q) { begin_frame(q); }

template <bool REFB> RT_FORCEINLINE void primary_ray(const RtCamera& cam, int x, int y, int W, int H, int aa, uint32_t& seed, float4& O, float4& D)
{
    if (cam.type == RT_CAM_PROJECTION) {
        float u = (float)x * (1.0f / (float)W);
        float v = (float)y * (1.0f / (float)H);
        if (aa) { u += rnd_float(seed) / (float)W; v += rnd_float(seed) / (float)H; }
        float4 P = add4(add4(ld4(cam.topLeft), muls(ld4(cam.horizontal), u)), muls(ld4(cam.vertical), v));
        float4 dir = normalize4<REFB>(sub4(P, ld4(cam.origin)));
        float4 focalPoint = add4(ld4(cam.origin), muls(dir, cam.focalLength));
        O = add4(ld4(cam.origin), muls(sub4(rnd_float3(seed), splat(0.5f)), cam.aperture));
        D = normalize4<REFB>(sub4(focalPoint, O));
    } else {
        float u = ((float)x - (float)W * .5f) * (2.f / (float)W);
        float v = ((float)y - (float)H * .5f) * (2.f / (float)H);
        if (aa) { u += rnd_float(seed) / (float)W; v += rnd_float(seed) / (float)H; }
        float r2 = u * u + v * v;
        if (r2 > 1.0f) { O = splat(0.0f); D = splat(0.0f); return; }
        float rr = sqrtf(r2);
        float psi = rr * cam.fov * kPi / 180.0f;
        float sinPsi = rt_sinf<REFB>(psi), cosPsi = rt_cosf<REFB>(psi);
        float sinAlpha = u / rr, cosAlpha = v / rr;
        D = sub4(add4(muls(ld4(cam.up), sinPsi * cosAlpha), muls(ld4(cam.right), sinPsi * sinAlpha)), muls(ld4(cam.forward), cosPsi));
        O = ld4(cam.origin);
    }
}
template <bool REFB>
__global__ __launch_bounds__(kBlock) void k_generate(DevQueues q, RtCamera cam, int aa, int beginFrame)
{
    const int i = blockIdx.x * kBlock + threadIdx.x;
    if (beginFrame && blockIdx.x == 0) begin_frame(q);
    if (threadIdx.x == 0) { q.tile[0][1 + blockIdx.x] = 0ull; if ((blockIdx.x & 63) == 0) { q.super[0][blockIdx.x >> 6] = 0ull; q.supAcc[0][blockIdx.x >> 6] = 0ull; } }
    if (i >= q.nPix) return;
    const int idx = q.firstPixel + i;
    uint32_t seed = q.seeds[i];
    float4 O, D;
    primary_ray<REFB>(cam, idx % q.width, idx / q.width, q.width, q.height, aa, seed, O, D);
    q.seeds[i] = seed;
    stnt4(&q.O[0][i], O); stnt4(&q.D[0][i], D); stnt4(&q.inten[0][i], splat(1.0f));
    stnt2(&q.meta[0][i], make_uint2((uint32_t)idx, kMetaLastSpec));
}

template <int ACCEL, int LAYOUT>
__global__ __launch_bounds__(kBlock) void k_extend(DevScene sc, DevQueues q, int bounce, int renderBVH)
{
    extern __shared__ uint32_t stk[];
    const int i = blockIdx.x * kBlock + threadIdx.x;
    const int n = q.nRays[bounce];
    WorkCtr wc = { 0, 0, 0, 0 };
    uint32_t rays = 0;
    if (i < n) {
        TRay r;
        world_ray(r, q.O[bounce & 1][i], q.D[bounce & 1][i], kFar);
        int steps = traverse_tlas<ACCEL, LAYOUT, false>(sc, r, stk, wc);
        rays = 1;
        q.hit[i] = mk4(r.t, __int_as_float(r.prim), r.u, r.v);
        if (q.steps) q.steps[i] = steps;
        if (renderBVH) q.accum[q.firstPixel + i] = splat((float)(uint32_t)steps / 255.f);
    }
    flush_counters(q.ctrExtend, rays, wc, stk);
}

#ifdef RT355_TAIL_PROBE
static constexpr int kTpWaves = 8192;
__device__ unsigned long long g_tp[9][kTpWaves][4];
#endif

RT_FORCEINLINE int xcd_pack(int n, int xcdRays, int xcdFirst, int& waves)
{
    const int wpb = kBlock / 64, wave = threadIdx.x >> 6;
    waves = gridDim.x * wpb;
    if (xcdRays <= 0 || (gridDim.x & 7u) != 0u) return blockIdx.x * wpb + wave;
    const int perXcd = (int)(gridDim.x >> 3) * kBlock;
    int nx = min(8, max(1, (n + xcdRays - 1) / xcdRays));
    while (nx < 8 && (long long)nx * perXcd < (long long)n) nx++;
    if (nx == 8) return blockIdx.x * wpb + wave;
    const int xcd = (int)(blockIdx.x + 8u - (uint32_t)xcdFirst) & 7;
    waves = (int)(gridDim.x >> 3) * nx * wpb;
    if (xcd >= nx) return -1;
    return ((int)(blockIdx.x >> 3) * nx + xcd) * wpb + wave;
}

struct SparseMap { int first, stride, per; };
RT_FORCEINLINE SparseMap sparse_map(int n, const PersistTune& t, int waveId)
{
    SparseMap m = { waveId, (int)gridDim.x * (kBlock / 64), 64 };
    if (t.xcdRays <= 0 && t.thin <= 0) return m;
    m.first = xcd_pack(n, t.xcdRays, t.xcdFirst, m.stride);
    if (t.thin > 0 && (long long)m.stride * t.thin >= (long long)n) m.per = max(1, (n + m.stride - 1) / m.stride);
    return m;
}

template <bool OCC> RT_FORCEINLINE bool primary_tiles(const DevQueues& q, int b0, int n)
{
    return !OCC && b0 == 0 && n == q.nPix && ((q.width | (q.nPix / q.width)) & 7) == 0;
}
RT_FORCEINLINE int tile_slot(const DevQueues& q, int tile, int lane)
{
    const int tilesX = q.width >> 3, ty = tile / tilesX, tx = tile - ty * tilesX;
    return ((ty << 3) + (lane >> 3)) * q.width + (tx << 3) + (lane & 7);
}

template <bool OCC> RT_FORCEINLINE int short_queue_slot(const DevQueues& q, int b0, int n, const PersistTune& t, int waveId, int lane)
{
    if (primary_tiles<OCC>(q, b0, n) && (long long)gridDim.x * kBlock >= (long long)q.nPix) return tile_slot(q, waveId, lane);
    if (b0 == 0 && n == q.nPix) return waveId * 64 + lane;
    const SparseMap m = sparse_map(n, t, waveId);
    return m.first < 0 || lane >= m.per ? n : m.first * m.per + lane;
}

struct QueueWindow { int first, n; int32_t* cursor; };
template <bool OCC> RT_FORCEINLINE QueueWindow queue_window(const DevQueues& q, int b0, int b1)
{
    const int first = OCC ? q.nShadow[b0] : 0;
    return { first, OCC ? q.nShadow[b1 + 1] - first : q.nRays[b0], q.cursor + (OCC ? (RT_MAX_BOUNCES + 2) + b0 : b0) };
}

struct OneInstance { float4 t0, t1, t2; uint32_t root; };
RT_FORCEINLINE OneInstance one_instance(const DevScene& sc)
{
    const uint32_t b = sc.tlas[0].BLASidx;
    const float* T = sc.blas[b].invT;
    return { mk4(T[0], T[1], T[2], T[3]), mk4(T[4], T[5], T[6], T[7]), mk4(T[8], T[9], T[10], T[11]), sc.rootEntry[b] };
}

template <bool OCC> RT_FORCEINLINE void queue_ray(TRay& r, const DevQueues& q, int b0, int qFirst, int idx, const OneInstance* inst = nullptr)
{
    float4 O, D; float tmax;
    if (OCC) { const float4 a = q.sA[qFirst + idx], b = q.sB[qFirst + idx]; O = a; D = b; tmax = a.w; }
    else { O = q.O[b0 & 1][idx]; D = q.D[b0 & 1][idx]; tmax = kFar; }
    if (inst) { object_space(r, mk4(O.x, O.y, O.z, 0.0f), mk4(D.x, D.y, D.z, 0.0f), inst->t0, inst->t1, inst->t2); reciprocal_dir(r); }
    else ray_from(r, O, D);
    no_hit(r, tmax);
}

template <bool OCC, bool STEPS>
RT_FORCEINLINE void store_result(const DevQueues& q, int qFirst, int idx, const TRay& r, int steps, bool occluded, int renderBVH)
{
    if (OCC) { if (occluded) q.sC[qFirst + idx] = splat(0.0f); }
    else {
        q.hit[idx] = mk4(r.t, __int_as_float(r.prim), r.u, r.v);
        if (STEPS) {
            if (q.steps) q.steps[idx] = steps;
            if (renderBVH) q.accum[q.firstPixel + idx] = splat((float)(uint32_t)steps / 255.f);
        }
    }
}

struct ChunkDealer {
    int next, end, round = 0;
    bool exhausted = false;
#ifdef RT355_TAIL_PROBE
    unsigned long long tpDry = 0;
#endif
    RT_FORCEINLINE ChunkDealer(int waveId, int chunk, int n) : next(min(waveId * chunk, n)), end(min(waveId * chunk + chunk, n)) {}
    RT_FORCEINLINE bool refill(bool idle, int& idx, uint32_t& dealt, const QueueWindow& w, const PersistTune& t, int nWaves, int waveId, int lane)
    {
        idx = -1;
        const unsigned long long idleMask = __ballot(idle);
        const int nIdle = __popcll(idleMask);
        if (nIdle == 64 && exhausted && next >= end) return false;
        if (nIdle < t.refill || (exhausted && next >= end)) return true;
        if (next >= end) {
            int c = 0;
            if (t.fixedChunks) { round++; c = round * nWaves * t.chunk + waveId * t.chunk; }
            else {
                if (lane == 0) c = atomicAdd(w.cursor, t.chunk);
                c = __shfl(c, 0, 64) + nWaves * t.chunk;
            }
            next = c; end = min(c + t.chunk, w.n);
            if (c >= w.n) { exhausted = true; next = end = 0; }
#ifdef RT355_TAIL_PROBE
            if (exhausted) tpDry = wall_clock64();
#endif
        }
        if (next < end) {
            const int i = next + __popcll(idleMask & ((1ull << lane) - 1ull));
            if (idle && i < end) idx = i;
            dealt += (uint32_t)min(nIdle, end - next);
            next = min(next + nIdle, end);
        }
        return true;
    }
};

template <bool OCC, bool STEPS>
RT_FORCEINLINE int node_event(const TRay& r, float tLight, float4 q0, float4 q1, float4 q2, float4 q3, uint32_t* stk, uint32_t& cur, uint32_t& sp, int& steps, bool& done)
{
    uint32_t e1 = pair_entry1(q3), e2 = pair_entry2(q3);
    int child = 0;
    if (OCC) {
        float x1, x2;
        const bool h1 = slab_any(r, pair_min1(q0, q1, q2), pair_max1(q0, q1, q2), x1);
        const bool h2 = slab_any(r, pair_min2(q0, q1, q2), pair_max2(q0, q1, q2), x2);
        if (h1 && h2) { const bool firstIs2 = x2 > x1; cur = firstIs2 ? e2 : e1; STK(sp) = firstIs2 ? e1 : e2; sp++; child = firstIs2 ? 2 : 1; }
        else if (h1 || h2) { cur = h1 ? e1 : e2; child = h1 ? 1 : 2; }
        else if (sp == 0) done = true;
        else cur = STK(--sp);
    } else {
        float d1 = slab(r, pair_min1(q0, q1, q2), pair_max1(q0, q1, q2));
        float d2 = slab(r, pair_min2(q0, q1, q2), pair_max2(q0, q1, q2));
        const bool swap = d1 > d2;
        if (swap) { float d = d1; d1 = d2; d2 = d; uint32_t e = e1; e1 = e2; e2 = e; }
        if (d1 >= tLight) {
            if (sp == 0) done = true;
            else cur = STK(--sp);
        } else {
            if (STEPS) steps++;
            cur = e1; child = swap ? 2 : 1;
            if (d2 < tLight) { STK(sp) = e2; sp++; if (STEPS) steps++; }
        }
    }
    return child;
}

static constexpr int kTopMaxLevels = 6;
RT_FORCEINLINE void fill_top(const DevScene& sc, uint32_t root, float4* top, int levels)
{
    const float4 absent = mk4(__uint_as_float(kLeafBit), __uint_as_float(kLeafBit), 0.0f, 0.0f);
    for (int l = 0; l < levels; l++) {
        const int n = 1 << l, t = (int)threadIdx.x;
        if (t < n) {
            const int s = n - 1 + t;
            uint32_t e = root;
            if (l > 0) { const float4 up = top[((s - 1) >> 1) * 4 + 3]; e = __float_as_uint((s & 1) ? up.x : up.y); }
            float4 q0 = splat(0.0f), q1 = q0, q2 = q0, q3 = absent;
            if (!(e & kLeafBit)) { const float4* p = sc.pairs + (size_t)e * 4; q0 = p[0]; q1 = p[1]; q2 = p[2]; q3 = p[3]; }
            float4* o = top + s * 4;
            o[0] = q0; o[1] = q1; o[2] = q2; o[3] = q3;
        }
        __syncthreads();
    }
}

template <bool OCC, bool STEPS>
RT_FORCEINLINE void top_descent(const DevQueues& q, const QueueWindow& w, int renderBVH, const float4* top, int levels, bool fresh, const TRay& r, float tLight,
                                uint32_t* stk, uint32_t& cur, uint32_t& sp, int& steps, int& slot, uint32_t& wNode, uint32_t& wNodeIss)
{
    const uint32_t nSlots = (1u << levels) - 1u;
    uint32_t ts = 0;
    bool in = fresh && nSlots != 0u && !(cur & kLeafBit);
    for (;;) {
        const unsigned long long m = __ballot(in);
        if (m == 0ull) break;
        wNode += (uint32_t)__popcll(m); if (STEPS) wNodeIss++;
        if (in) {
            const float4* p = top + ts * 4;
            const float4 q0 = p[0], q1 = p[1], q2 = p[2], q3 = p[3];
            bool done = false;
            const int child = node_event<OCC, STEPS>(r, tLight, q0, q1, q2, q3, stk, cur, sp, steps, done);
            if (done) { store_result<OCC, STEPS>(q, w.first, slot, r, steps, false, renderBVH); slot = -1; }
            ts = 2u * ts + (uint32_t)child;
            in = child != 0 && ts < nSlots && !(cur & kLeafBit);
        }
    }
}

template <bool OCC, bool COH, bool BVH4 = false>
RT_FORCEINLINE void trace_short_queue(const DevScene& sc, const DevQueues& q, int b0, const QueueWindow& w, int renderBVH, const OneInstance& one,
                                      uint32_t* stk, int waveId, int lane, const PersistTune& tune)
{
    WorkCtr wc = { 0, 0, 0, 0 };
    uint32_t rays = 0;
    const int idx = short_queue_slot<OCC>(q, b0, w.n, tune, waveId, lane);
    if (idx < w.n) {
        TRay r;
        queue_ray<OCC>(r, q, b0, w.first, idx, &one);
        rays = 1; wc.inst = 1;
        const int st = BVH4 ? traverse_bvh4_packed<OCC>(sc, r, one.root, stk, wc)
                     : COH ? traverse_bvh2_packed_coherent(sc, r, one.root, stk, wc) : traverse_bvh2_packed<OCC>(sc, r, one.root, stk, wc);
        store_result<OCC, true>(q, w.first, idx, r, st, st == -1, renderBVH);
    }
    flush_counters(OCC ? q.ctrConnect : q.ctrExtend, rays, wc, stk);
}


template <bool OCC, bool COH = false, bool STEPS = false, bool TOP = false>
__global__ __launch_bounds__(kBlock) void k_trace_persist(DevScene sc, DevQueues q, int b0, int b1, int renderBVH, PersistTune tune)
{
    const int kInner = tune.inner, kLeafK = tune.leafK;
    extern __shared__ uint32_t stk[];
    const int lane = threadIdx.x & 63;
    const QueueWindow w = queue_window<OCC>(q, b0, b1);
    const OneInstance one = one_instance(sc);

    WorkCtr wc = { 0, 0, 0, 0 };
    uint32_t rays = 0;
    uint32_t wRays = 0, wNode = 0, wPrim = 0, wNodeIss = 0, wLeafIss = 0;
    TRay r; r.t = 0; r.prim = -1; r.u = r.v = 0; r.ox = r.oy = r.oz = r.dx = r.dy = r.dz = r.rx = r.ry = r.rz = 0;
    uint32_t cur = 0, sp = 0;
    int slot = -1, steps = 0;
    float tLight = 0;
    const int nWaves = gridDim.x * (kBlock / 64), waveId = blockIdx.x * (kBlock / 64) + (threadIdx.x >> 6);
#ifdef RT355_TAIL_PROBE
    const unsigned long long tp0 = wall_clock64();
#define TAIL_PROBE_EXIT(tpDry) if (lane == 0 && waveId < kTpWaves) { unsigned long long* p = g_tp[OCC ? 8 : b0][waveId]; p[0] = tp0; p[1] = tpDry; p[2] = wall_clock64(); p[3] = rays; }
#endif
    if (w.n <= nWaves * 64) {
        trace_short_queue<OCC, COH>(sc, q, b0, w, renderBVH, one, stk, waveId, lane, tune);
#ifdef RT355_TAIL_PROBE
        TAIL_PROBE_EXIT(0ull)
#endif
        return;
    }
    float4* const top = reinterpret_cast<float4*>(stk + tune.topBase);
    if (TOP) fill_top(sc, one.root, top, tune.topLevels);
    ChunkDealer deal(waveId, tune.chunk, w.n);
    for (;;) {
        int idx;
        if (!deal.refill(slot < 0, idx, wRays, w, tune, nWaves, waveId, lane)) break;
        if (idx >= 0) { queue_ray<OCC>(r, q, b0, w.first, idx, &one); tLight = r.t; cur = one.root; sp = 0; steps = 0; slot = idx; }
        if (TOP) top_descent<OCC, STEPS>(q, w, renderBVH, top, tune.topLevels, idx >= 0, r, tLight, stk, cur, sp, steps, slot, wNode, wNodeIss);
#pragma unroll 1
        for (int it = 0; it < kInner; it++) {
            const bool act = slot >= 0, atLeaf = act && (cur & kLeafBit) != 0u;
            const unsigned long long lm = __ballot(atLeaf), im = __ballot(act && !atLeaf);
            if ((lm | im) == 0ull) break;
            const bool doLeaf = im == 0ull || __popcll(lm) >= kLeafK;
            bool done = false, occluded = false;
            if (!doLeaf) { wNode += (uint32_t)__popcll(im); if (STEPS) wNodeIss++; }
            if (doLeaf) {
                wPrim += (uint32_t)__popcll(lm); if (STEPS) wLeafIss++;
                if (atLeaf) {
                    const uint32_t first = leaf_first(cur), count = leaf_count(cur);
                    test_tri_packed(sc, first, r);
                    if (OCC && r.t < tLight) { done = true; occluded = true; }
                    else if (count > 1) cur = leaf_rest(first, count);
                    else if (sp == 0) done = true;
                    else cur = STK(--sp);
                }
            } else if (act && !atLeaf) {
                const float4* p = sc.pairs + (size_t)cur * 4;
                const float4 q0 = p[0], q1 = p[1], q2 = p[2], q3 = p[3];
                node_event<OCC, STEPS>(r, tLight, q0, q1, q2, q3, stk, cur, sp, steps, done);
            }
            if (done) { store_result<OCC, STEPS>(q, w.first, slot, r, steps, occluded, renderBVH); slot = -1; }
        }
    }
#ifdef RT355_TAIL_PROBE
    TAIL_PROBE_EXIT(deal.tpDry)
#endif
    if (lane == 0) { rays = wRays; wc.inst = wRays; wc.node = wNode; wc.prim = wPrim; if (STEPS) { wc.nodeIss = wNodeIss; wc.leafIss = wLeafIss; wc.evNode = wNode; wc.evPrim = wPrim; } }
    flush_counters(OCC ? q.ctrConnect : q.ctrExtend, rays, wc, stk);
}

template <bool SPILL> RT_FORCEINLINE void stk_push(uint32_t* stk, const DevQueues& q, uint32_t gl, uint32_t& sp, uint32_t e)
{
    if (!SPILL || sp < q.stackCap) stk[sp * kBlock + threadIdx.x] = e;
    else q.spill[(size_t)(sp - q.stackCap) * q.spillStride + gl] = e;
    sp++;
}
template <bool SPILL> RT_FORCEINLINE uint32_t stk_pop(const uint32_t* stk, const DevQueues& q, uint32_t gl, uint32_t& sp)
{
    --sp;
    return (!SPILL || sp < q.stackCap) ? stk[sp * kBlock + threadIdx.x] : q.spill[(size_t)(sp - q.stackCap) * q.spillStride + gl];
}
RT_FORCEINLINE void inst_enter(const DevScene& sc, const DevQueues& q, uint32_t* stk, TRay& r, uint32_t& cur, uint32_t sp, uint32_t& spBase,
                               bool& inInst, float& tLight)
// ... 589 lines not shown
        if (NEE) ext.lastSpec = true;
    } else {
        const float4 albedo = albedo_of<REFB>(sc, tab, prim, mat, mc, ray);
        const float4 BRDF = muls(albedo, kInvPi);
        if (NEE && sc.nLights > 0) {
            uint32_t li = f2u_gpu(floorf(rnd_abs(seed) * (float)sc.nLights));
            if (li >= (uint32_t)sc.nLights) li = (uint32_t)sc.nLights - 1;
            float4 l0, l1, l2, l3, l4, l5;
            if (tab.on) { const uint32_t r = li * (uint32_t)kShadeLightRows; l0 = tab_row(tab, r); l1 = tab_row(tab, r + 1); l2 = tab_row(tab, r + 2); l3 = tab_row(tab, r + 3); l4 = tab_row(tab, r + 4); l5 = tab_row(tab, r + 5); }
            else { const float4* LR = sc.lightRecs + (size_t)li * 8; l0 = LR[0]; l1 = LR[1]; l2 = LR[2]; l3 = LR[3]; l4 = LR[4]; l5 = LR[5]; }
            asm volatile("" : : "v"(l0.x), "v"(l1.x), "v"(l2.x), "v"(l3.x), "v"(l4.x), "v"(l5.x));
            const int ltype = __float_as_int(l4.x);
            const float larea = l4.y;
            float4 pl, Nl;
            if (ltype == RT_PRIM_SPHERE) {
                float theta = rnd_abs(seed) * 2.0f * kPi;
                float u = rnd_abs(seed) * 2.0f - 1.0f;
                float pre = sqrtf(1 - u * u);
                float x = rt_cosf<REFB>(theta) * pre, y = rt_sinf<REFB>(theta) * pre;
                pl = add4(muls(mk4(x, y, u, 0.0f), l1.x), l0);
                Nl = muls(sub4(pl, l0), l1.z);
            } else {
                float u1 = rnd_abs(seed), u2 = rnd_abs(seed);
                if (u1 + u2 > 1) { u1 = 1 - u1; u2 = 1 - u2; }
                float4 a = sub4(l1, l0), b = sub4(l2, l0);
                pl = add4(add4(l0, muls(a, u1)), muls(b, u2));
                Nl = ltype == RT_PRIM_PLANE ? l0 : l3;
            }
            float4 dirToLight = sub4(pl, ray.I);
            float dist = length4<REFB>(dirToLight);
            float4 L = muls(dirToLight, 1 / dist);
            float dotNL = dot4(ray.N, L);
            if (dotNL > 0 && dot4(Nl, neg4(L)) > 0) {
                float4 sInt = muls(ray.inten, (float)sc.nLights);
                float solidAngle = dot4(Nl, neg4(L)) * larea * (1 / (dist * dist));
                float4 lightColor = l5;
                float4 Ld = muls(mul4(muls(lightColor, solidAngle), BRDF), dotNL);
                float4 color = firefly<REFB>(var.fireflies, mul4(Ld, sInt));
                float4 so = add4(ray.I, muls(L, kEps));
                sh.a = mk4(so.x, so.y, so.z, dist - 2 * kEps);
                sh.b = mk4(L.x, L.y, L.z, __int_as_float(ray.pixel));
                sh.c = color;
                sh.valid = true;
            }
        }
        if (var.rr) {
            float rr_p = survival_prob(albedo);
            if (rr_p < rnd_float(seed)) return splat(0.0f);
            ray.inten = muls(ray.inten, 1 / rr_p);
        }
        float4 refl = sample_dir<REFB>(var.sampling, ray.N, seed);
        float dotNR = dot4(ray.N, refl);
        float I_PDF = var.sampling == RT_SAMPLING_HEMISPHERE ? 2 * kPi : dotNR * kPi;
        ext.O = add4(ray.I, muls(refl, kEps));
        ext.D = refl;
        if (NEE) ext.inten = muls(muls(mul4(ray.inten, BRDF), I_PDF), dotNR);
        else     ext.inten = mul4(ray.inten, muls(muls(BRDF, I_PDF), dotNR));
        ext.bounces = ray.bounces + 1; ext.inside = ray.inside; ext.lastSpec = false; ext.valid = true;
    }
    return splat(0.0f);
}

static constexpr unsigned long long kTileAgg = 1ull << 62, kTilePrefix = 2ull << 62, kTilePrefixZero = 2ull << 62;
RT_FORCEINLINE unsigned long long tile_pack(unsigned long long flag, uint32_t e, uint32_t s) { return flag | ((unsigned long long)e << 31) | (unsigned long long)s; }
RT_FORCEINLINE uint32_t tile_ext(unsigned long long v) { return (uint32_t)((v >> 31) & 0x7fffffffull); }
RT_FORCEINLINE uint32_t tile_sh(unsigned long long v) { return (uint32_t)(v & 0x7fffffffull); }

static constexpr uint32_t kSpinLimit = 1u << 22;
RT_FORCEINLINE unsigned long long wait_word(const unsigned long long* p, unsigned long long needFlag , int32_t* fault, int32_t what = 1)
{
    unsigned long long v = __hip_atomic_load(p, __ATOMIC_RELAXED, __HIP_MEMORY_SCOPE_AGENT);
    uint32_t spins = 0;
    while (needFlag == 2ull ? (v >> 62) != 2ull : (v >> 62) == 0ull) {
        if (++spins > kSpinLimit || ((spins & 1023u) == 0u && __hip_atomic_load(fault, __ATOMIC_RELAXED, __HIP_MEMORY_SCOPE_AGENT) != 0)) { atomicCAS(fault, 0, what); return kTilePrefixZero; }
        if (spins < 4) __builtin_amdgcn_s_sleep(2); else __builtin_amdgcn_s_sleep(32);
        v = __hip_atomic_load(p, __ATOMIC_RELAXED, __HIP_MEMORY_SCOPE_AGENT);
    }
    return v;
}

static_assert(RT_MAX_BOUNCES < 0x40 && kMetaInside == 0x100u && kMetaLastSpec == 0x200u, "park_meta packs meta.y into one byte");
RT_FORCEINLINE uint8_t park_meta(uint32_t y) { return (uint8_t)((y & 0x3fu) | ((y & (kMetaInside | kMetaLastSpec)) >> 2)); }
RT_FORCEINLINE uint32_t unpark_meta(uint8_t b) { return ((uint32_t)b & 0x3fu) | (((uint32_t)b & 0xc0u) << 2); }
template <bool NEE, int TILE, bool REFB>
__global__ __launch_bounds__(TILE, 4) void k_shade(DevScene sc, DevQueues q, DevVariant var, int bounce)
{
    __shared__ uint32_t sWaveE[2][TILE / 64], sWaveS[2][TILE / 64], sBaseE, sBaseS;
    enum { P_EXT_O, P_EXT_D, P_EXT_I, P_SH_A, P_SH_C, P_ROWS4 = NEE ? 5 : 3 };
    __shared__ float4 sPark4[P_ROWS4 * TILE + kShadeTableRows];
    __shared__ float2 sShB[NEE ? TILE : 1];
    __shared__ uint2 sPixZ[TILE];
    __shared__ uint8_t sExtM[TILE];
    auto park_slot = [] { uint32_t s = threadIdx.x; asm volatile("" : "+v"(s)); return s; };
    const int cur = bounce & 1, nxt = cur ^ 1;
    unsigned long long* state = q.tile[cur];
    unsigned long long* const* super = q.super;
    const int n = q.nRays[bounce];
    if (n <= 0) {
        if (blockIdx.x == 0 && threadIdx.x == 0) { q.nRays[bounce + 1] = 0; q.nShadow[bounce + 1] = q.nShadow[bounce]; }
        return;
    }
    const uint32_t numTiles = (uint32_t)((n + TILE - 1) / TILE);
    const int wave = threadIdx.x >> 6, lane = threadIdx.x & 63;
    const int shadowBase = q.nShadow[bounce];

    auto drain = [&](uint32_t t, int pp, unsigned long long em, unsigned long long sm, bool extValid, bool shValid) {
        if (wave == 0) {
            uint32_t aggE = 0, aggS = 0;
#pragma unroll
            for (int w = 0; w < TILE / 64; w++) { aggE += sWaveE[pp][w]; aggS += sWaveS[pp][w]; }
            const uint32_t sup = t >> 6, inSup = t & 63u;
            unsigned long long v = 0ull;
            if ((uint32_t)lane < inSup) v = wait_word(&state[1 + (sup << 6) + (uint32_t)lane], 0ull, q.fault, 0x10000000 | (int32_t)((sup << 6) + (uint32_t)lane));
            else if (lane == 63 && sup > 0) v = wait_word(&super[cur][sup - 1], 2ull, q.fault, 0x20000000 | (int32_t)(sup - 1));
            const unsigned long long vp = __shfl(v, 63, 64);
            const uint32_t preE = sup > 0 ? tile_ext(vp) : 0u, preS = sup > 0 ? tile_sh(vp) : 0u;
            uint32_t inE = (uint32_t)lane < inSup ? tile_ext(v) : 0u, inS = (uint32_t)lane < inSup ? tile_sh(v) : 0u;
#pragma unroll
            for (int off = 32; off > 0; off >>= 1) { inE += __shfl_xor(inE, off, 64); inS += __shfl_xor(inS, off, 64); }
            if (lane == 0) {
                sBaseE = preE + inE; sBaseS = preS + inS;
                if (t == numTiles - 1) { q.nRays[bounce + 1] = (int)(preE + inE + aggE); q.nShadow[bounce + 1] = shadowBase + (int)(preS + inS + aggS); }
            }
        }
        __syncthreads();
        uint32_t baseE = sBaseE, baseS = sBaseS + (uint32_t)shadowBase;
        for (int w = 0; w < wave; w++) { baseE += sWaveE[pp][w]; baseS += sWaveS[pp][w]; }
        const unsigned long long below = (1ull << lane) - 1ull;
        const uint32_t slot = park_slot();
        if (extValid) {
            const uint32_t dst = baseE + (uint32_t)__popcll(em & below);
            q.O[nxt][dst] = sPark4[P_EXT_O * TILE + slot]; q.D[nxt][dst] = sPark4[P_EXT_D * TILE + slot]; q.inten[nxt][dst] = sPark4[P_EXT_I * TILE + slot];
            q.meta[nxt][dst] = make_uint2(sPixZ[slot].x, unpark_meta(sExtM[slot]));
        }
        if (NEE && shValid) {
            const uint32_t dst = baseS + (uint32_t)__popcll(sm & below);
            const float2 bxy = sShB[slot]; const uint2 pz = sPixZ[slot];
            q.sA[dst] = sPark4[P_SH_A * TILE + slot]; q.sB[dst] = mk4(bxy.x, bxy.y, __uint_as_float(pz.y), __uint_as_float(pz.x)); q.sC[dst] = sPark4[P_SH_C * TILE + slot];
        }
        __syncthreads();
    };

#ifdef RT355_SHADE_TIMING
    long long tShade = 0, tDrain = 0, tBegin = wall_clock64(); int nT = 0;
#endif
    bool pend = false, pExt = false, pSh = false;
    uint32_t pTile = 0;
    unsigned long long pEm = 0ull, pSm = 0ull;
    int par = 0;
    struct TileIn { float4 hit, O, D, inten; uint2 meta; uint32_t seed; };
    auto fetch = [&](uint32_t t, TileIn& in) {
        const int j = (int)t * TILE + threadIdx.x;
        if (t < numTiles && j < n) {
            in.hit = ldnt4(&q.hit[j]); in.meta = ldnt2(&q.meta[cur][j]); in.O = ldnt4(&q.O[cur][j]); in.D = ldnt4(&q.D[cur][j]); in.inten = ldnt4(&q.inten[cur][j]);
            in.seed = q.seeds[j];
        }
    };
    __shared__ uint32_t sTicket;
    const uint32_t cls = blockIdx.x % (uint32_t)kTicketClasses;
    int32_t* ticket = q.shadeTicket + ((size_t)bounce * kTicketClasses + cls) * kTicketStride;
    uint32_t tkNext = 0;
    const ShadeTab tab = { (lds_rows)(sPark4 + P_ROWS4 * TILE), (uint32_t)kShadeLightRows * (uint32_t)sc.nLights, var.shadeTables != 0 && shade_tables_fit(sc.nLights, sc.nMats) };
    const uint32_t tabRows = tab.on ? tab.mat0 + (uint32_t)kShadeMatRows * (uint32_t)sc.nMats : 0u;
    float4 tabRow = splat(0.0f);
    if (threadIdx.x < tabRows) {
        const uint32_t r = threadIdx.x, m = r - tab.mat0;
        if (r < tab.mat0) tabRow = sc.lightRecs[(size_t)(r / kShadeLightRows) * 8 + r % kShadeLightRows];
        else tabRow = reinterpret_cast<const float4*>(sc.mats + m / kShadeMatRows)[m % kShadeMatRows ? m % kShadeMatRows + 1 : 0];
    }
    if (threadIdx.x == 0) sTicket = (uint32_t)atomicAdd(ticket, 1);
    __syncthreads();
    uint32_t tile = sTicket * (uint32_t)kTicketClasses + cls;
    TileIn in;
    fetch(tile, in);
    if (threadIdx.x < tabRows) sPark4[P_ROWS4 * TILE + threadIdx.x] = tabRow;
    __syncthreads();
    for (; tile < numTiles; par ^= 1) {
        const int i = (int)tile * TILE + threadIdx.x;
        if (threadIdx.x == 0) {
            q.tile[nxt][1 + tile] = 0ull;
            tkNext = (uint32_t)atomicAdd(ticket, 1);
        }
#ifdef RT355_SHADE_TIMING
        const long long c0 = wall_clock64();
#endif

        bool extValid = false, shValid = false;
        ExtRay ext; ext.valid = false;
        ShadowOut sh; sh.valid = false;
        uint2 extMeta = make_uint2(0u, 0u);
        if (i < n) {
            const float4 hit = in.hit;
            const uint2 meta = in.meta;
            SRay ray;
            ray.O = in.O; ray.D = in.D; ray.inten = in.inten;
            ray.t = hit.x; ray.prim = __float_as_int(hit.y); ray.u = hit.z; ray.v = hit.w;
            ray.pixel = (int)meta.x; ray.bounces = (int)(meta.y & kMetaBounceMask);
            ray.inside = (meta.y & kMetaInside) != 0; ray.lastSpec = (meta.y & kMetaLastSpec) != 0;
            if (ray.prim == -1) {
                float4 c = mul4(ray.inten, mk4(0.0784f, 0.0941f, 0.3215f, 0.0f));
                q.accum[ray.pixel] = add4(q.accum[ray.pixel], c);
            } else {
                ray.I = add4(ray.O, muls(ray.D, ray.t));
                const float4 rec = sc.shadeRecs[ray.prim];
                asm volatile("" : : "v"(rec.x), "v"(rec.w));
                const uint32_t tag = __float_as_uint(rec.w);
                ray.matIdx = (int)(tag & 0x07ffffffu);
                ray.N = (tag >> 28) == RT_PRIM_SPHERE ? prim_normal(sc.prims + ray.prim, ray.I)
                                                      : mk4(rec.x, rec.y, rec.z, (tag & 0x08000000u) ? -0.0f : 0.0f);
                if (dot4(ray.N, neg4(ray.D)) < 0) ray.N = muls(ray.N, -1.0f);
                uint32_t seed = in.seed;
                float4 color = shade_hit<NEE, REFB>(sc, tab, var, ray, seed, ext, sh);
                q.seeds[i] = seed;
                color = firefly<REFB>(var.fireflies, color);
                if (color.x != 0.0f || color.y != 0.0f || color.z != 0.0f || color.w != 0.0f)
                    q.accum[ray.pixel] = add4(q.accum[ray.pixel], color);
                if (ext.valid && ext.bounces <= RT_MAX_BOUNCES) {
                    extValid = true;
                    extMeta = make_uint2((uint32_t)ray.pixel, (uint32_t)ext.bounces | (ext.inside ? kMetaInside : 0u) | (ext.lastSpec ? kMetaLastSpec : 0u));
                }
                shValid = sh.valid;
            }
        }
        const unsigned long long em = __ballot(extValid), sm = __ballot(shValid);
        if (lane == 0) { sWaveE[par][wave] = (uint32_t)__popcll(em); sWaveS[par][wave] = (uint32_t)__popcll(sm); }
        if (threadIdx.x == 0) sTicket = tkNext;
        __syncthreads();
        if (wave == 0) {
            uint32_t aggE = 0, aggS = 0;
#pragma unroll
            for (int w = 0; w < TILE / 64; w++) { aggE += sWaveE[par][w]; aggS += sWaveS[par][w]; }
            const uint32_t sup = tile >> 6;
            unsigned long long acc = 0ull;
            if (lane == 0) {
                __hip_atomic_store(&state[1 + tile], tile_pack(kTileAgg, aggE, aggS), __ATOMIC_RELAXED, __HIP_MEMORY_SCOPE_AGENT);
                if ((tile & 63u) == 0u) { super[nxt][sup] = 0ull; q.supAcc[nxt][sup] = 0ull; }
                acc = __hip_atomic_fetch_add(&q.supAcc[cur][sup], (1ull << 40) | ((unsigned long long)aggE << 20) | (unsigned long long)aggS,
                                             __ATOMIC_RELAXED, __HIP_MEMORY_SCOPE_AGENT);
            }
            acc = __shfl(acc, 0, 64);
            if ((acc >> 40) == 63ull) {
                const uint32_t totE = (uint32_t)((acc >> 20) & 0xfffffull) + aggE, totS = (uint32_t)(acc & 0xfffffull) + aggS;
                uint32_t preE = 0, preS = 0;
                if (sup > 0) {
                    if (lane == 0) __hip_atomic_store(&super[cur][sup], tile_pack(kTileAgg, totE, totS), __ATOMIC_RELAXED, __HIP_MEMORY_SCOPE_AGENT);
                    int top = (int)sup - 1;
                    for (;;) {
                        const int tt = top - lane;
                        unsigned long long v = kTilePrefix;
                        if (tt >= 0) v = wait_word(&super[cur][tt], 0ull, q.fault, 0x30000000 | tt);
                        const unsigned long long isPre = __ballot((v >> 62) == 2ull);
                        const int stop = isPre ? __ffsll((long long)isPre) - 1 : 64;
                        uint32_t e = lane <= stop ? tile_ext(v) : 0u, s2 = lane <= stop ? tile_sh(v) : 0u;
#pragma unroll
                        for (int off = 32; off > 0; off >>= 1) { e += __shfl_xor(e, off, 64); s2 += __shfl_xor(s2, off, 64); }
                        preE += e; preS += s2;
                        if (isPre) break;
                        top -= 64;
                    }
                }
                if (lane == 0) __hip_atomic_store(&super[cur][sup], tile_pack(kTilePrefix, preE + totE, preS + totS), __ATOMIC_RELAXED, __HIP_MEMORY_SCOPE_AGENT);
            }
        }
#ifdef RT355_SHADE_TIMING
        const long long c1 = wall_clock64();
#endif
        const uint32_t nextTile = sTicket * (uint32_t)kTicketClasses + cls;
        TileIn inNext;
        fetch(nextTile, inNext);
        if (pend) drain(pTile, par ^ 1, pEm, pSm, pExt, pSh);
        else __syncthreads();
        in = inNext;
#ifdef RT355_SHADE_TIMING
        tShade += c1 - c0; tDrain += wall_clock64() - c1; nT++;
#endif
        const uint32_t slot = park_slot();
        if (extValid) { sPark4[P_EXT_O * TILE + slot] = ext.O; sPark4[P_EXT_D * TILE + slot] = ext.D; sPark4[P_EXT_I * TILE + slot] = ext.inten; sExtM[slot] = park_meta(extMeta.y); }
        if (NEE && shValid) { sPark4[P_SH_A * TILE + slot] = sh.a; sShB[slot] = make_float2(sh.b.x, sh.b.y); sPark4[P_SH_C * TILE + slot] = sh.c; }
        if (extValid || shValid) sPixZ[slot] = make_uint2(shValid ? __float_as_uint(sh.b.w) : extMeta.x, __float_as_uint(sh.b.z));
        pend = true; pTile = tile; pEm = em; pSm = sm; pExt = extValid; pSh = shValid;
        tile = nextTile;
    }
    if (pend) {
        __syncthreads();
        drain(pTile, par ^ 1, pEm, pSm, pExt, pSh);
    }
#ifdef RT355_SHADE_TIMING
    if (threadIdx.x == 0 && (blockIdx.x & 127) == 5 && bounce <= 1)
        printf("shade b%d block %d tiles %d: shade %lld drain %lld total %lld (x10 ns)\n", bounce, blockIdx.x, nT, tShade, tDrain, wall_clock64() - tBegin);
#endif
}

template <int ACCEL, int LAYOUT>
__global__ __launch_bounds__(kBlock) void k_connect(DevScene sc, DevQueues q, int b0, int b1)
// ... 167 lines not shown
```

### magr_ray_tracer_amd/csrc/trav_common.h

```cpp
#pragma once
#include <algorithm>
#include <cstdio>
#include <cstdlib>
#include "../../include/rt355.h"

namespace rt355dev {

struct PersistTune {
    int chunk, refill, inner, leafK;
    int fixedChunks;
    int flat = 0;
    int xcdRays = 0, xcdFirst = 0;
    int thin = 0;
    int topLevels = 0, topBase = 0;
};

enum Traversal {
    TRAV_NESTED,
    TRAV_BVH2,
    TRAV_TLAS,
    TRAV_TLAS_SPILL,
    TRAV_BVH4,
    TRAV_BVH4_TLAS,
    TRAV_BVH4_TLAS_SPILL,
};
static inline bool persistent(int trav) { return trav != TRAV_NESTED; }
static inline bool spill_trav(int trav) { return trav == TRAV_TLAS_SPILL || trav == TRAV_BVH4_TLAS_SPILL; }
static inline bool bvh4_tlas_trav(int trav) { return trav == TRAV_BVH4_TLAS || trav == TRAV_BVH4_TLAS_SPILL; }
static inline bool tlas_trav(int trav) { return trav == TRAV_TLAS || trav == TRAV_TLAS_SPILL || bvh4_tlas_trav(trav); }

constexpr int kAdmitAnySgpr = 6, kAdmit96Sgpr = 7;
constexpr int kFitSeven = 22, kBackupWords = 10, kSpillCap = kFitSeven - kBackupWords;
constexpr int kTopLevelsExtend = 6, kTopLevelsConnect = 6;
constexpr int kColumnLanes = 256, kTopLevelsMax = 6;

static inline size_t stack_bytes(int stackEntries) { return (size_t)stackEntries * kColumnLanes * sizeof(uint32_t); }
static inline size_t top_bytes(int levels) { return levels > 0 ? (((size_t)1 << levels) - 1) * 64 : 0; }
static inline int tlas_stack_entries(int stackEntries, int tlasDepth) { return stackEntries + tlasDepth + 1; }
static inline int tlas_lds_entries(int trav, int spillCap, int stackEntries, int tlasDepth) { return spill_trav(trav) ? spillCap : tlas_stack_entries(stackEntries, tlasDepth); }
static inline size_t tlas_column_bytes(int entries) { return (size_t)(entries + kBackupWords) * kColumnLanes * sizeof(uint32_t); }

struct TravFacts {
    int accel = 0, extend_variant = 0, persist_blocks_per_cu = 0;
    int layout = 0, singleBlas = 0, tlasDepth = 0, nInterior = 0, nQuads = 0, stackEntries = 0;
    int sharedMemPerBlock = 0;
    int xcdFirst = 0;
};

struct TravKnobs {
    bool spillCapSet = false; int spillCap = 0;
    bool noSpill = false;
    bool coherentSet = false; int coherent = 0;
    bool tuneSet = false; int tune[4] = {};
    int tuneBlocks = 0;
    bool fixedChunksSet = false; int fixedChunks[2] = {};
    bool tuneConnectSet = false; int tuneConnect[4] = {};
    bool topLevelsSet = false; int topLevels[2] = {};
    bool flatSet = false; int flat[2] = {};
    bool xcdRaysSet = false; int xcdRays = 0;
    bool thinSet = false; int thin = 0;
    int connectBlocks = 0;
};

static inline TravKnobs read_trav_knobs()
{
    TravKnobs k;
    auto tune_ok = [](int a, int b, int c, int l) { return a > 0 && b > 0 && b <= 64 && c > 0 && l > 0 && l <= 64; };
    if (const char* t = getenv("RT355_SPILL_CAP")) { const int v = atoi(t); if (v >= 6 && v <= 64) { k.spillCap = v; k.spillCapSet = true; } }
    if (const char* t = getenv("RT355_NO_SPILL")) k.noSpill = atoi(t) != 0;
    if (const char* t = getenv("RT355_COHERENT")) { k.coherent = atoi(t); k.coherentSet = true; }
    if (const char* t = getenv("RT355_TUNE")) {
        int a = 0, b = 0, c = 0, l = 0, d = 0;
        const int n = sscanf(t, "%d,%d,%d,%d,%d", &a, &b, &c, &l, &d);
        if (n >= 4 && tune_ok(a, b, c, l)) { k.tune[0] = a; k.tune[1] = b; k.tune[2] = c; k.tune[3] = l; k.tuneSet = true; }
        if (n == 5 && d > 0) k.tuneBlocks = d;
    }
    if (const char* t = getenv("RT355_FIXED_CHUNKS")) { int a = 0, b = 0; if (sscanf(t, "%d,%d", &a, &b) == 2) { k.fixedChunks[0] = a; k.fixedChunks[1] = b; k.fixedChunksSet = true; } }
    if (const char* t = getenv("RT355_TUNE_CONNECT")) {
        int a = 0, b = 0, c = 0, l = 0;
        if (sscanf(t, "%d,%d,%d,%d", &a, &b, &c, &l) == 4 && tune_ok(a, b, c, l)) { k.tuneConnect[0] = a; k.tuneConnect[1] = b; k.tuneConnect[2] = c; k.tuneConnect[3] = l; k.tuneConnectSet = true; }
    }
    if (const char* t = getenv("RT355_TOP_LEVELS")) {
        int a = 0, b = 0;
        const int n = sscanf(t, "%d,%d", &a, &b);
        if (n == 1) b = a;
        if (n >= 1 && a >= 0 && a <= kTopLevelsMax && b >= 0 && b <= kTopLevelsMax) { k.topLevels[0] = a; k.topLevels[1] = b; k.topLevelsSet = true; }
    }
    if (const char* t = getenv("RT355_TLAS_FLAT")) { int a = 0, b = 0; if (sscanf(t, "%d,%d", &a, &b) == 2) { k.flat[0] = a; k.flat[1] = b; k.flatSet = true; } }
    if (const char* t = getenv("RT355_XCD_RAYS")) { k.xcdRays = std::max(0, atoi(t)); k.xcdRaysSet = true; }
    if (const char* t = getenv("RT355_THIN")) { k.thin = std::min(64, std::max(0, atoi(t))); k.thinSet = true; }
    if (const char* t = getenv("RT355_CONNECT_BLOCKS")) { const int d = atoi(t); if (d > 0) k.connectBlocks = d; }
    return k;
}

struct TravPlan {
    int trav = TRAV_NESTED;
    int spillCap = kSpillCap;
    int coherent = 1;
    PersistTune tune{}, tuneConnect{}, tune4{};
    bool topAuto = false;
    int tuneBlocks = 0, connectBlocks = 0;
};

static inline TravPlan plan_traversal(const TravFacts& f, const TravKnobs& k)
{
    TravPlan p;
    const int entries = tlas_stack_entries(f.stackEntries, f.tlasDepth);
    p.trav = TRAV_NESTED;
    if (f.layout == 1 && f.extend_variant != 2) {
        if (f.singleBlas) p.trav = f.accel == RT_ACCEL_BVH2 ? TRAV_BVH2 : (f.accel == RT_ACCEL_BVH4 ? TRAV_BVH4 : TRAV_NESTED);
        else if (f.accel == RT_ACCEL_BVH2 && f.extend_variant != 4 && f.tlasDepth <= 8 && f.nInterior < (1 << 29)) p.trav = TRAV_TLAS;
    }
    if (f.layout == 1 && f.extend_variant == 6 && f.accel == RT_ACCEL_BVH4 && !f.singleBlas && f.tlasDepth <= 8 && f.nQuads < (1 << 29)) p.trav = TRAV_BVH4_TLAS;
    p.spillCap = k.spillCapSet ? k.spillCap : kSpillCap;
    const bool forceSpill = k.spillCapSet;
    if (p.trav == TRAV_TLAS && (entries > kFitSeven || forceSpill) && entries > p.spillCap && !k.noSpill) p.trav = TRAV_TLAS_SPILL;
    if (p.trav == TRAV_TLAS && entries > RT_BVH4_STACK + 9) p.trav = TRAV_NESTED;
    if (p.trav == TRAV_BVH4_TLAS) {
        const size_t lds = (size_t)std::max(0, f.sharedMemPerBlock);
        const bool fits = tlas_column_bytes(entries) <= lds;
        const bool canSpill = !k.noSpill && entries > p.spillCap && tlas_column_bytes(p.spillCap) <= lds;
        if ((entries > kFitSeven || forceSpill || !fits) && canSpill) p.trav = TRAV_BVH4_TLAS_SPILL;
        else if (!fits) p.trav = TRAV_NESTED;
    }
    p.coherent = k.coherentSet ? k.coherent : 1;

    p.tune = PersistTune{ 112, 24, 6, 8, 0 }; p.tuneConnect = PersistTune{ 128, 32, 6, 16, 0 }; p.tune4 = PersistTune{ 64, 20, 6, 8, 0 };
    if (f.persist_blocks_per_cu > 0) {
        p.tune.leafK = 16;
    } else {
        p.tune.fixedChunks = p.tuneConnect.fixedChunks = p.tune4.fixedChunks = 1;
    }
    if (k.tuneSet) p.tune = p.tuneConnect = p.tune4 = PersistTune{ k.tune[0], k.tune[1], k.tune[2], k.tune[3], 0 };
    p.tuneBlocks = k.tuneBlocks; p.connectBlocks = k.connectBlocks;
    if (k.fixedChunksSet) { p.tune.fixedChunks = p.tune4.fixedChunks = k.fixedChunks[0]; p.tuneConnect.fixedChunks = k.fixedChunks[1]; }
    if (k.tuneConnectSet) p.tuneConnect = PersistTune{ k.tuneConnect[0], k.tuneConnect[1], k.tuneConnect[2], k.tuneConnect[3], 0 };
    p.tune.topLevels = p.tuneConnect.topLevels = 0;
    if (p.trav == TRAV_BVH2) {
        p.tune.topLevels = kTopLevelsExtend; p.tuneConnect.topLevels = kTopLevelsConnect;
        p.topAuto = true;
        if (k.topLevelsSet) { p.tune.topLevels = k.topLevels[0]; p.tuneConnect.topLevels = k.topLevels[1]; p.topAuto = false; }
    }
    if (tlas_trav(p.trav)) {
        p.tune.flat = p.tune4.flat = 1; p.tuneConnect.flat = 0;
        if (k.flatSet) { p.tune.flat = p.tune4.flat = k.flat[0]; p.tuneConnect.flat = k.flat[1]; }
    }
    p.tune.xcdRays = p.tuneConnect.xcdRays = p.tune4.xcdRays = k.xcdRaysSet ? k.xcdRays : 1024;
    p.tune.xcdFirst = p.tuneConnect.xcdFirst = p.tune4.xcdFirst = f.xcdFirst;
    p.tune.thin = p.tuneConnect.thin = p.tune4.thin = k.thinSet ? k.thin : 16;
    return p;
}

struct ShadeKnobs {
    bool tablesSet = false; int tables = 0;
    int tile = 0;
    int perCU = 0;
};
static inline ShadeKnobs read_shade_knobs()
{
    ShadeKnobs k;
    if (const char* t = getenv("RT355_SHADE_TABLES")) { k.tables = atoi(t) != 0; k.tablesSet = true; }
    if (const char* t = getenv("RT355_SHADE_TILE")) { const int v = atoi(t); if (v == 256 || v == 512) k.tile = v; }
    if (const char* t = getenv("RT355_SHADE_PER_CU")) { const int v = atoi(t); if (v > 0 && v <= 16) k.perCU = v; }
    return k;
}

}
```

### magr_ray_tracer_amd/renderer.py

```python
import ctypes as C

import numpy as np

from . import _lib


class RtError(RuntimeError):
    code = None


def traversal_plan(facts):
    lib = _lib.device_lib()
    f, p = np.zeros((), dtype=_lib.TraversalFacts), np.zeros((), dtype=_lib.TraversalPlan)
    for n, v in facts.items():
        f[n] = v
    if lib.rt_debug_traversal_plan(f.ctypes.data_as(C.c_void_p), p.ctypes.data_as(C.c_void_p)) != 0:
        raise RtError(lib.rt_last_error().decode())
    out = {n: int(p[n]) for n in ("trav", "spillCap", "coherent", "tuneBlocks", "connectBlocks")}
    out["topAuto"] = bool(p["topAuto"])
    for n in ("tune", "tuneConnect", "tune4"):
        out[n] = dict(zip(_lib.TUNE_FIELDS, (int(v) for v in p[n])))
    return out


# ... 318 lines not shown

    def update_geometry(self, first=0, prims=None, positions=None, indices=None, instances=None):
        args, keep, st = _update_geometry_args(first, prims, positions, indices, instances)
        self._chk_code(self._lib.rt_update_geometry(self._h, *args))
        return _update_dict(st)

    def rebuild_geometry(self, first=0, prims=None, positions=None, indices=None, instances=None, builder="sah", alpha=None, **lbvh_options):
        args, keep, st = _rebuild_geometry_args(first, prims, positions, indices, instances, builder, lbvh_options, alpha)
        self._chk_code(self._lib.rt_rebuild_geometry(self._h, *args))
        return _rebuild_dict(st)

    def rebuild_geometry_ranges(self, plan, first=0, prims=None, positions=None, indices=None, instances=None, alpha=None, **lbvh_options):
        args, keep, st = _geometry_ranges_args(plan, first, prims, positions, indices, instances, lbvh_options, alpha)
        self._chk_code(self._lib.rt_rebuild_geometry_ranges(self._h, *args))
        return _rebuild_dict(st)

    def ranges_info(self):
        r = np.zeros((), _lib.RangesInfo)
        self._chk(self._lib.rt_ranges_info(self._h, _lib.ptr(r)))
        return {n: int(r[n]) for n in _lib.RANGES_INFO_FIELDS}

    def blas_blocks(self):
        n = C.c_int32(0)
        self._chk_code(self._lib.rt_scene_blas_blocks(self._h, C.byref(n), None, None, None, None, None, 0))
        a = np.zeros((5, max(n.value, 1)), np.int32)
        self._chk_code(self._lib.rt_scene_blas_blocks(self._h, C.byref(n), *[C.c_void_p(a[i].ctypes.data) for i in range(5)], n.value))
        return [dict(prim_first=int(a[0, k]), prim_count=int(a[1, k]), nodes=int(a[2, k]), idx_slots=int(a[3, k]), compact=bool(a[4, k]))
                for k in range(n.value)]

    def resize_scene(self, prims, range_counts, inst_range=None, instances=None, builder="sah", alpha=None, **lbvh_options):
        args, keep, st = _resize_args(prims, range_counts, inst_range, instances, builder, lbvh_options, alpha)
        self._chk_code(self._lib.rt_resize_scene(self._h, *args))
        return _rebuild_dict(st)

    def update_materials(self, mats=None, texels=None, tex_first=0, n_texels=None, prim_mat=None, prim_first=0):
        args, keep, st = _materials_args(mats, texels, tex_first, n_texels, prim_mat, prim_first)
        self._chk_code(self._lib.rt_update_materials(self._h, *args))
        return _materials_dict(st)

    def refit_info(self):
        r = np.zeros((), _lib.RefitInfo)
        self._chk(self._lib.rt_refit_info(self._h, _lib.ptr(r)))
        return {n: int(r[n]) for n in r.dtype.names}

    def rebuild_allocations(self):
        n = C.c_int64(0)
        self._chk(self._lib.rt_debug_rebuild_allocations(self._h, C.byref(n)))
        return n.value

    def scene_array(self, name):
        which = {**_lib.SCENE_ARRAYS, **_lib.SCENE_ARRAYS_BVH4, **_lib.SCENE_ARRAYS_RESIZE, **_lib.SCENE_ARRAYS_MATERIALS}[name]
        n = C.c_int64(0)
        self._chk(self._lib.rt_debug_get_scene_array(self._h, which, None, 0, C.byref(n)))
        out = np.zeros(n.value, dtype=np.uint8)
        if n.value:
            self._chk(self._lib.rt_debug_get_scene_array(self._h, which, _lib.ptr(out), n.value, C.byref(n)))
        return out

    def kernel_info(self):
        k = np.zeros((), dtype=_lib.KernelInfo)
        self._chk(self._lib.rt_kernel_info(self._h, k.ctypes.data_as(C.c_void_p)))
        return {n: int(k[n]) for n in k.dtype.names}

    def top_levels(self):
        e, c = C.c_int32(0), C.c_int32(0)
        self._chk(self._lib.rt_top_levels(self._h, C.byref(e), C.byref(c)))
        return int(e.value), int(c.value)

    def traversal_facts(self):
        f = np.zeros((), dtype=_lib.TraversalFacts)
        self._chk(self._lib.rt_debug_traversal_facts(self._h, f.ctypes.data_as(C.c_void_p)))
        return {n: int(f[n]) for n in f.dtype.names}

    def shade_footprint(self):
        b, t = C.c_int32(0), C.c_int32(0)
        self._chk(self._lib.rt_shade_footprint(self._h, C.byref(b), C.byref(t)))
        return int(b.value), int(t.value)

    def shade_tables(self):
        r, s = C.c_int32(0), C.c_int32(0)
        self._chk(self._lib.rt_shade_tables(self._h, C.byref(r), C.byref(s)))
        return int(r.value), bool(s.value)

    @property
    def builtins(self):
        rc = self._lib.rt_builtins(self._h)
        if rc < 0:
            self._chk(rc)
        return int(rc)

    def extend_kernel_name(self):
        k = self.kernel_info()
        if k["persist4"] == 3:
            return "k_trace_persist4_tlas<false, false, true> (LDS stack of %d entries per lane, deeper entries in global memory)" % k["stack_entries"]
        if k["persist4"] == 2:
            return "k_trace_persist4_tlas<false> (bounce 0: its one-ray-per-lane branch)"
        if k["persist4"]:
            return "k_trace_persist4<false>"
        if k["persist"] == 3:
            return "k_trace_persist_tlas<false, false, true> (LDS stack of %d entries per lane, deeper entries in global memory)" % k["stack_entries"]
        if k["persist"] == 2:
            return "k_trace_persist_tlas<false> (bounce 0: its one-ray-per-lane branch)"
        if k["persist"]:
            return "k_trace_persist<false> (bounce 0: <false, true>, node records of wave-uniform visits through the scalar cache)"
        return "k_extend<%s, %d>" % ("RT_ACCEL_BVH4" if self.accel == _lib.ACCEL_BVH4 else "RT_ACCEL_BVH2", k["layout"])

    def set_seeds(self, seeds):
        s = np.ascontiguousarray(seeds, dtype=np.uint32)
        self._chk_code(self._lib.rt_set_seeds(self._h, _lib.ptr(s), s.size))

    def seed_default(self):
        self._chk(self._lib.rt_seed_default(self._h))

    def get_seeds(self):
        s = np.zeros(self.npix, dtype=np.uint32)
        self._chk(self._lib.rt_get_seeds(self._h, _lib.ptr(s), s.size))
        return s

    def bind_accum(self, tensor):
        assert tensor.is_cuda and tensor.is_contiguous() and tensor.numel() == self.width * self.height * 4
        self._keep = tensor
        self._chk(self._lib.rt_bind_accum(self._h, C.c_void_p(tensor.data_ptr())))

    def reset(self):
        self._chk(self._lib.rt_reset(self._h))

    def render(self, cam, frames=1, antiAliasing=1, renderBVH=0):
        s = np.zeros((), dtype=_lib.Settings)
        s["antiAliasing"], s["renderBVH"] = antiAliasing, renderBVH
        c = np.ascontiguousarray(cam)
        self._chk(self._lib.rt_render(self._h, c.ctypes.data_as(C.c_void_p), s.ctypes.data_as(C.c_void_p), int(frames)))

    def synchronize(self):
        self._chk(self._lib.rt_synchronize(self._h))

    def focus(self, x, y, cam):
        t = C.c_float(0)
        c = np.ascontiguousarray(cam)
        self._chk(self._lib.rt_focus(self._h, int(x), int(y), c.ctypes.data_as(C.c_void_p), C.byref(t)))
        return np.float32(t.value)

    def read_accum(self):
        out = np.zeros((self.height, self.width, 4), dtype=np.float32)
        self._chk(self._lib.rt_read_accum(self._h, _lib.ptr(out)))
        return out

    def write_accum(self, accum):
        a = np.ascontiguousarray(accum, dtype=np.float32)
        assert a.shape == (self.height, self.width, 4)
        self._chk(self._lib.rt_write_accum(self._h, _lib.ptr(a)))

    def save_checkpoint(self, path, frames):
        np.savez_compressed(path, accum=self.read_accum(), seeds=self.get_seeds(), frames=np.int32(frames),
                            dims=np.array([self.width, self.height, self.y0, self.y1], np.int32))

    def load_checkpoint(self, path):
        g = np.load(path)
        assert tuple(g["dims"]) == (self.width, self.height, self.y0, self.y1), "checkpoint was taken with another frame/band"
        accum = g["accum"]
        assert accum.shape == (self.height, self.width, 4)
        self.set_seeds(g["seeds"])
        self.write_accum(accum)
        return int(g["frames"])

    def postproc(self, frames, vignette=0.0, gamma=0.9, chromatic=0.0):
        f = np.zeros((self.height, self.width, 4), dtype=np.float32)
# ... 374 lines not shown
```

Baseline: 1079.

## Fuse primary ray generation into bounce-0 extend and shade kernels

Result: faster. 1092 (median of 6 runs) (+1.2%).

```diff
diff --git a/include/rt355.h b/include/rt355.h
--- a/include/rt355.h
+++ b/include/rt355.h
@@ -91,6 +91,7 @@
 int rt_debug_traversal_facts(RtCtx* ctx, RtTraversalFacts* out);
 int rt_shade_footprint(RtCtx* ctx, int32_t* ldsBytes, int32_t* traversalBeside);
 int rt_shade_tables(RtCtx* ctx, int32_t* capacityRows, int32_t* staged);
+int rt_primary_fused(RtCtx* ctx, int32_t* fused);
 
 int rt_create(const RtConfig* cfg, RtCtx** out);
 int rt_destroy(RtCtx* ctx);
diff --git a/magr_ray_tracer_amd/_lib.py b/magr_ray_tracer_amd/_lib.py
--- a/magr_ray_tracer_amd/_lib.py
+++ b/magr_ray_tracer_amd/_lib.py
@@ -126,7 +126,7 @@
 assert RebuildStats.itemsize == 96
 
 DEVICE_SYMBOLS = [
-    "rt_last_error", "rt_device_count", "rt_kernel_info", "rt_builtins", "rt_top_levels", "rt_shade_footprint", "rt_shade_tables", "rt_create", "rt_destroy", "rt_upload_scene", "rt_share_scene", "rt_set_seeds", "rt_seed_default",
+    "rt_last_error", "rt_device_count", "rt_kernel_info", "rt_builtins", "rt_top_levels", "rt_shade_footprint", "rt_shade_tables", "rt_primary_fused", "rt_create", "rt_destroy", "rt_upload_scene", "rt_share_scene", "rt_set_seeds", "rt_seed_default",
     "rt_get_seeds", "rt_bind_accum", "rt_accum_device_ptr", "rt_stream", "rt_reset", "rt_render", "rt_synchronize", "rt_focus",
     "rt_read_accum", "rt_write_accum", "rt_postproc", "rt_read_counters", "rt_reset_counters", "rt_read_stage_times", "rt_reset_stage_times", "rt_set_profile",
     "rt_stage_begin_frame", "rt_stage_generate", "rt_stage_extend", "rt_stage_shade", "rt_stage_connect",
@@ -202,6 +202,7 @@
         lib.rt_debug_traversal_facts.argtypes = [vp, vp]
         lib.rt_shade_footprint.argtypes = [vp, C.POINTER(i32), C.POINTER(i32)]
         lib.rt_shade_tables.argtypes = [vp, C.POINTER(i32), C.POINTER(i32)]
+        lib.rt_primary_fused.argtypes = [vp, C.POINTER(i32)]
         lib.rt_destroy.argtypes = [vp]
         lib.rt_upload_scene.argtypes = [vp, vp, i32, vp, i32, vp, i32, vp, i32, vp, i32, vp, i32, vp, i32, vp, i32]
         lib.rt_upload_scene_bvh2.argtypes = lib.rt_upload_scene.argtypes
diff --git a/magr_ray_tracer_amd/csrc/ctx.h b/magr_ray_tracer_amd/csrc/ctx.h
--- a/magr_ray_tracer_amd/csrc/ctx.h
+++ b/magr_ray_tracer_amd/csrc/ctx.h
@@ -43,8 +43,12 @@
     int shadeTile = rt355dev::kTile;
     int shadeGrid = 1024;
     void (*kGenerate)(rt355dev::DevQueues, RtCamera, int, int) = nullptr;
-    void (*kShade)(rt355dev::DevScene, rt355dev::DevQueues, rt355dev::DevVariant, int) = nullptr;
+    void (*kShade)(rt355dev::DevScene, rt355dev::DevQueues, rt355dev::DevVariant, rt355dev::ShadeArg<false>) = nullptr;
     void (*kFocus)(rt355dev::DevScene, RtCamera, int, int, int, int, float*) = nullptr;
+    enum { PRIMARY_PLAIN, PRIMARY_COHERENT, PRIMARY_BVH4, PRIMARY_KINDS };
+    void (*kTracePrimary[PRIMARY_KINDS])(rt355dev::DevScene, rt355dev::DevQueues, RtCamera, int, int, rt355dev::PersistTune) = {};
+    void (*kShadePrimary)(rt355dev::DevScene, rt355dev::DevQueues, rt355dev::DevVariant, rt355dev::ShadeArg<true>) = nullptr;
+    bool fusePrimary = false;
 };
 
 static inline dim3 grid_for(int n) { return dim3((unsigned)std::max(1, (n + rt355dev::kBlock - 1) / rt355dev::kBlock)); }
diff --git a/magr_ray_tracer_amd/csrc/rt355.hip b/magr_ray_tracer_amd/csrc/rt355.hip
--- a/magr_ray_tracer_amd/csrc/rt355.hip
+++ b/magr_ray_tracer_amd/csrc/rt355.hip
@@ -27,6 +27,10 @@
     ctx->kGenerate = k_generate<REFB>;
     ctx->kShade = nee ? (small ? k_shade<true, 256, REFB> : k_shade<true, kTile, REFB>) : (small ? k_shade<false, 256, REFB> : k_shade<false, kTile, REFB>);
     ctx->kFocus = ctx->cfg.accel == RT_ACCEL_BVH4 ? k_focus<RT_ACCEL_BVH4, REFB> : k_focus<RT_ACCEL_BVH2, REFB>;
+    ctx->kTracePrimary[RtCtx::PRIMARY_PLAIN] = k_trace_primary<REFB, false, false>;
+    ctx->kTracePrimary[RtCtx::PRIMARY_COHERENT] = k_trace_primary<REFB, true, false>;
+    ctx->kTracePrimary[RtCtx::PRIMARY_BVH4] = k_trace_primary<REFB, false, true>;
+    ctx->kShadePrimary = nee ? (small ? k_shade<true, 256, REFB, true> : k_shade<true, kTile, REFB, true>) : (small ? k_shade<false, 256, REFB, true> : k_shade<false, kTile, REFB, true>);
 }
 static void choose_builtin_kernels(RtCtx* ctx)
 {
@@ -93,6 +97,15 @@
     return RT_OK;
 }
 
+extern "C" int rt_primary_fused(RtCtx* ctx, int32_t* fused)
+{
+    if (!ctx || !fused) return fail(RT_E_INVALID, "rt_primary_fused: null argument");
+    if (!ctx->sceneLoaded) return fail(RT_E_INVALID, "rt_primary_fused: no scene uploaded");
+    if (const int rc = sync_scene_config(ctx)) return rc;
+    *fused = ctx->fusePrimary ? 1 : 0;
+    return RT_OK;
+}
+
 static void free_bag(std::vector<void*>& bag) { for (void* p : bag) (void)hipFree(p); bag.clear(); }
 
 static void scene_release(RtCtx* ctx)
@@ -122,14 +135,17 @@
 
 using PersistKernel = void (*)(DevScene, DevQueues, int, int, int, PersistTune);
 using NestedKernel = void (*)(DevScene, DevQueues, int, int);
+using PrimaryKernel = void (*)(DevScene, DevQueues, RtCamera, int, int, PersistTune);
 struct TraceLaunch {
     PersistKernel persist = nullptr;
     NestedKernel nested = nullptr;
+    PrimaryKernel primary = nullptr;
     dim3 grid;
     size_t lds = 0;
     PersistTune tune{};
 };
-static TraceLaunch trace_launch(const RtCtx* c, int stage, int bounce, bool steps, int rays, int topLevels = -1 )
+static TraceLaunch trace_launch(const RtCtx* c, int stage, int bounce, bool steps, int rays, int topLevels = -1 ,
+                                bool primary = false )
 {
     TraceLaunch L;
     L.grid = grid_for(rays);
@@ -153,6 +169,7 @@
             L.grid = dim3(c->persistGrid);
         }
         else if (c->cfg.extend_variant == 5) L.nested = k_extend<RT_ACCEL_BVH2, 1>;
+        else if (primary && c->fusePrimary) L.primary = c->kTracePrimary[c->coherent ? RtCtx::PRIMARY_COHERENT : RtCtx::PRIMARY_PLAIN];
         else L.persist = c->coherent ? k_trace_persist<false, true> : (steps ? k_trace_persist<false, false, true> : k_trace_persist<false>);
         if (top) { L.tune.topBase = c->facts.stackEntries * kBlock; L.lds += top_bytes(L.tune.topLevels); }
         break;
@@ -160,6 +177,7 @@
         L.tune = connect ? c->tuneConnect : c->tune4;
         L.persist = connect ? k_trace_persist4<true> : k_trace_persist4<false>;
         if (connect || bounce > 0) L.grid = dim3(connect ? c->persistGridConnect : c->persistGrid);
+        else if (primary && c->fusePrimary) { L.persist = nullptr; L.primary = c->kTracePrimary[RtCtx::PRIMARY_BVH4]; }
         break;
     case TRAV_TLAS:
     case TRAV_TLAS_SPILL: {
@@ -410,6 +428,7 @@
     ctx->trav = p.trav; ctx->spillCap = p.spillCap; ctx->coherent = p.coherent;
     ctx->tune = p.tune; ctx->tuneConnect = p.tuneConnect; ctx->tune4 = p.tune4;
     ctx->tuneBlocks = p.tuneBlocks; ctx->connectBlocks = p.connectBlocks;
+    ctx->fusePrimary = p.fusePrimary;
 }
 static int fit_top_tables(RtCtx* ctx, bool topAuto)
 {
@@ -848,7 +867,22 @@
     HIPCHK(hipGetLastError());
     return RT_OK;
 }
-extern "C" int rt_stage_shade(RtCtx* ctx, int32_t bounce)
+static int extend_primary(RtCtx* ctx, const RtCamera* cam, const RtSettings* s, int renderBVH)
+{
+    frame_state_reset(ctx);
+    ctx->queued = true;
+    const TraceLaunch L = trace_launch(ctx, ST_EXTEND, 0, false, ctx->nPix, -1, true);
+    if (!L.primary) return fail(RT_E_INVALID, "rt_render: no fused primary launch for this context's traversal");
+    LAUNCH(ctx, ST_EXTEND, L.primary, L.grid, L.lds, ctx->sc, ctx->q, *cam, s ? s->antiAliasing : 1, renderBVH, L.tune);
+    HIPCHK(hipGetLastError());
+    ctx->primaryRays += (uint64_t)ctx->nPix;
+    ctx->generated = true;
+    ctx->cursorUsed[0] = true;
+    return RT_OK;
+}
+static int stage_shade(RtCtx* ctx, int32_t bounce, const RtCamera* primaryCam, int aa);
+extern "C" int rt_stage_shade(RtCtx* ctx, int32_t bounce) { return stage_shade(ctx, bounce, nullptr, 0); }
+static int stage_shade(RtCtx* ctx, int32_t bounce, const RtCamera* primaryCam, int aa)
 {
     int rc = need_scene(ctx, "rt_stage_shade"); if (rc) return rc;
     ctx->queued = true;
@@ -862,7 +896,8 @@
     }
     const int tileSz = ctx->shadeTile;
     const dim3 sg((unsigned)std::max(1, std::min(ctx->shadeGrid, (ctx->nPix + tileSz - 1) / tileSz)));
-    LAUNCHB(ctx, ST_SHADE, ctx->kShade, sg, tileSz, 0, ctx->sc, ctx->q, ctx->var, bounce);
+    if (primaryCam) LAUNCHB(ctx, ST_SHADE, ctx->kShadePrimary, sg, tileSz, 0, ctx->sc, ctx->q, ctx->var, ShadeArg<true>{ { *primaryCam, aa } });
+    else LAUNCHB(ctx, ST_SHADE, ctx->kShade, sg, tileSz, 0, ctx->sc, ctx->q, ctx->var, ShadeArg<false>{ bounce });
     ctx->shadeRun[bounce] = true;
     HIPCHK(hipGetLastError());
     return RT_OK;
@@ -1020,12 +1055,14 @@
     HIPCHK(hipSetDevice(ctx->cfg.device));
     const bool nee = ctx->cfg.shading == RT_SHADING_NEE, rr = ctx->cfg.russian_roulette != 0;
     const int renderBVH = settings ? settings->renderBVH : 0;
+    const bool fused = ctx->fusePrimary;
+    const int aa = settings ? settings->antiAliasing : 1;
     for (int f = 0; f < frames; f++) {
-        if ((rc = generate(ctx, cam, settings, 1))) return rc;
+        if ((rc = fused ? extend_primary(ctx, cam, settings, renderBVH) : generate(ctx, cam, settings, 1))) return rc;
         for (int b = 0; b < ctx->cfg.max_bounces; b++) {
-            if ((rc = rt_stage_extend(ctx, b, renderBVH))) return rc;
+            if (b > 0 || !fused) if ((rc = rt_stage_extend(ctx, b, renderBVH))) return rc;
             if (renderBVH) break;
-            if ((rc = rt_stage_shade(ctx, b))) return rc;
+            if ((rc = stage_shade(ctx, b, fused && b == 0 ? cam : nullptr, aa))) return rc;
             if (!rr && nee) if ((rc = rt_stage_connect(ctx, b, b))) return rc;
         }
         if (rr && nee && !renderBVH) if ((rc = rt_stage_connect(ctx, 0, ctx->cfg.max_bounces - 1))) return rc;
diff --git a/magr_ray_tracer_amd/csrc/rt355_dev.h b/magr_ray_tracer_amd/csrc/rt355_dev.h
--- a/magr_ray_tracer_amd/csrc/rt355_dev.h
+++ b/magr_ray_tracer_amd/csrc/rt355_dev.h
@@ -57,6 +57,9 @@
 };
 static constexpr int kTicketClasses = 1, kTicketStride = 1024, kCursorWords = 2 * (RT_MAX_BOUNCES + 2);
 struct DevVariant { int32_t shading, sampling, accel, rr, fireflies, maxBounces, shadeTables ; };
+struct PrimaryArgs { RtCamera cam; int aa; };
+template <bool PRIMARY> struct ShadeArg { int bounce; };
+template <> struct ShadeArg<true> { static constexpr int bounce = 0; PrimaryArgs gen; };
 static constexpr int kCtrCols = 9;
 static constexpr int kTile = 512;
 
diff --git a/magr_ray_tracer_amd/csrc/rt355_kernels.h b/magr_ray_tracer_amd/csrc/rt355_kernels.h
--- a/magr_ray_tracer_amd/csrc/rt355_kernels.h
+++ b/magr_ray_tracer_amd/csrc/rt355_kernels.h
@@ -451,6 +451,7 @@
 
 template <bool REFB> RT_FORCEINLINE void primary_ray(const RtCamera& cam, int x, int y, int W, int H, int aa, uint32_t& seed, float4& O, float4& D)
 {
+    float4 o = splat(0.0f), d = splat(0.0f);
     if (cam.type == RT_CAM_PROJECTION) {
         float u = (float)x * (1.0f / (float)W);
         float v = (float)y * (1.0f / (float)H);
@@ -458,21 +459,23 @@
         float4 P = add4(add4(ld4(cam.topLeft), muls(ld4(cam.horizontal), u)), muls(ld4(cam.vertical), v));
         float4 dir = normalize4<REFB>(sub4(P, ld4(cam.origin)));
         float4 focalPoint = add4(ld4(cam.origin), muls(dir, cam.focalLength));
-        O = add4(ld4(cam.origin), muls(sub4(rnd_float3(seed), splat(0.5f)), cam.aperture));
-        D = normalize4<REFB>(sub4(focalPoint, O));
+        o = add4(ld4(cam.origin), muls(sub4(rnd_float3(seed), splat(0.5f)), cam.aperture));
+        d = normalize4<REFB>(sub4(focalPoint, o));
     } else {
         float u = ((float)x - (float)W * .5f) * (2.f / (float)W);
         float v = ((float)y - (float)H * .5f) * (2.f / (float)H);
         if (aa) { u += rnd_float(seed) / (float)W; v += rnd_float(seed) / (float)H; }
         float r2 = u * u + v * v;
-        if (r2 > 1.0f) { O = splat(0.0f); D = splat(0.0f); return; }
-        float rr = sqrtf(r2);
-        float psi = rr * cam.fov * kPi / 180.0f;
-        float sinPsi = rt_sinf<REFB>(psi), cosPsi = rt_cosf<REFB>(psi);
-        float sinAlpha = u / rr, cosAlpha = v / rr;
-        D = sub4(add4(muls(ld4(cam.up), sinPsi * cosAlpha), muls(ld4(cam.right), sinPsi * sinAlpha)), muls(ld4(cam.forward), cosPsi));
-        O = ld4(cam.origin);
-    }
+        if (!(r2 > 1.0f)) {
+            float rr = sqrtf(r2);
+            float psi = rr * cam.fov * kPi / 180.0f;
+            float sinPsi = rt_sinf<REFB>(psi), cosPsi = rt_cosf<REFB>(psi);
+            float sinAlpha = u / rr, cosAlpha = v / rr;
+            d = sub4(add4(muls(ld4(cam.up), sinPsi * cosAlpha), muls(ld4(cam.right), sinPsi * sinAlpha)), muls(ld4(cam.forward), cosPsi));
+            o = ld4(cam.origin);
+        }
+    }
+    O = o; D = d;
 }
 template <bool REFB>
 __global__ __launch_bounds__(kBlock) void k_generate(DevQueues q, RtCamera cam, int aa, int beginFrame)
@@ -573,14 +576,27 @@
     return { mk4(T[0], T[1], T[2], T[3]), mk4(T[4], T[5], T[6], T[7]), mk4(T[8], T[9], T[10], T[11]), sc.rootEntry[b] };
 }
 
+RT_FORCEINLINE void new_ray(TRay& r, const float4& O, const float4& D, float tmax, const OneInstance* inst)
+{
+    if (inst) { object_space(r, mk4(O.x, O.y, O.z, 0.0f), mk4(D.x, D.y, D.z, 0.0f), inst->t0, inst->t1, inst->t2); reciprocal_dir(r); }
+    else ray_from(r, O, D);
+    no_hit(r, tmax);
+}
 template <bool OCC> RT_FORCEINLINE void queue_ray(TRay& r, const DevQueues& q, int b0, int qFirst, int idx, const OneInstance* inst = nullptr)
 {
     float4 O, D; float tmax;
     if (OCC) { const float4 a = q.sA[qFirst + idx], b = q.sB[qFirst + idx]; O = a; D = b; tmax = a.w; }
     else { O = q.O[b0 & 1][idx]; D = q.D[b0 & 1][idx]; tmax = kFar; }
-    if (inst) { object_space(r, mk4(O.x, O.y, O.z, 0.0f), mk4(D.x, D.y, D.z, 0.0f), inst->t0, inst->t1, inst->t2); reciprocal_dir(r); }
-    else ray_from(r, O, D);
-    no_hit(r, tmax);
+    new_ray(r, O, D, tmax, inst);
+}
+template <bool REFB> RT_FORCEINLINE void primary_queue_ray(TRay& r, const DevQueues& q, const RtCamera& cam, int aa, int keepSeed, int idx, const OneInstance* inst)
+{
+    const int pix = q.firstPixel + idx;
+    uint32_t seed = q.seeds[idx];
+    float4 O, D;
+    primary_ray<REFB>(cam, pix % q.width, pix / q.width, q.width, q.height, aa, seed, O, D);
+    if (keepSeed) q.seeds[idx] = seed;
+    new_ray(r, O, D, kFar, inst);
 }
 
 template <bool OCC, bool STEPS>
@@ -705,16 +721,17 @@
     }
 }
 
-template <bool OCC, bool COH, bool BVH4 = false>
+template <bool OCC, bool COH, bool BVH4 = false, bool PRIMARY = false, bool REFB = false>
 RT_FORCEINLINE void trace_short_queue(const DevScene& sc, const DevQueues& q, int b0, const QueueWindow& w, int renderBVH, const OneInstance& one,
-                                      uint32_t* stk, int waveId, int lane, const PersistTune& tune)
+                                      uint32_t* stk, int waveId, int lane, const PersistTune& tune, const RtCamera* cam = nullptr, int aa = 0)
 {
     WorkCtr wc = { 0, 0, 0, 0 };
     uint32_t rays = 0;
     const int idx = short_queue_slot<OCC>(q, b0, w.n, tune, waveId, lane);
     if (idx < w.n) {
         TRay r;
-        queue_ray<OCC>(r, q, b0, w.first, idx, &one);
+        if (PRIMARY) primary_queue_ray<REFB>(r, q, *cam, aa, renderBVH, idx, &one);
+        else queue_ray<OCC>(r, q, b0, w.first, idx, &one);
         rays = 1; wc.inst = 1;
         const int st = BVH4 ? traverse_bvh4_packed<OCC>(sc, r, one.root, stk, wc)
                      : COH ? traverse_bvh2_packed_coherent(sc, r, one.root, stk, wc) : traverse_bvh2_packed<OCC>(sc, r, one.root, stk, wc);
@@ -723,6 +740,16 @@
     flush_counters(OCC ? q.ctrConnect : q.ctrExtend, rays, wc, stk);
 }
 
+template <bool REFB, bool COH, bool BVH4>
+__global__ __launch_bounds__(kBlock) void k_trace_primary(DevScene sc, DevQueues q, RtCamera cam, int aa, int renderBVH, PersistTune tune)
+{
+    extern __shared__ uint32_t stk[];
+    if (blockIdx.x == 0) begin_frame(q);
+    if (threadIdx.x == 0) { q.tile[0][1 + blockIdx.x] = 0ull; if ((blockIdx.x & 63) == 0) { q.super[0][blockIdx.x >> 6] = 0ull; q.supAcc[0][blockIdx.x >> 6] = 0ull; } }
+    const QueueWindow w = { 0, q.nPix, q.cursor };
+    const OneInstance one = one_instance(sc);
+    trace_short_queue<false, COH, BVH4, true, REFB>(sc, q, 0, w, renderBVH, one, stk, blockIdx.x * (kBlock / 64) + (threadIdx.x >> 6), threadIdx.x & 63, tune, &cam, aa);
+}
 
 template <bool OCC, bool COH = false, bool STEPS = false, bool TOP = false>
 __global__ __launch_bounds__(kBlock) void k_trace_persist(DevScene sc, DevQueues q, int b0, int b1, int renderBVH, PersistTune tune)
@@ -1478,9 +1505,10 @@
 static_assert(RT_MAX_BOUNCES < 0x40 && kMetaInside == 0x100u && kMetaLastSpec == 0x200u, "park_meta packs meta.y into one byte");
 RT_FORCEINLINE uint8_t park_meta(uint32_t y) { return (uint8_t)((y & 0x3fu) | ((y & (kMetaInside | kMetaLastSpec)) >> 2)); }
 RT_FORCEINLINE uint32_t unpark_meta(uint8_t b) { return ((uint32_t)b & 0x3fu) | (((uint32_t)b & 0xc0u) << 2); }
-template <bool NEE, int TILE, bool REFB>
-__global__ __launch_bounds__(TILE, 4) void k_shade(DevScene sc, DevQueues q, DevVariant var, int bounce)
-{
+template <bool NEE, int TILE, bool REFB, bool PRIMARY = false>
+__global__ __launch_bounds__(TILE, 4) void k_shade(DevScene sc, DevQueues q, DevVariant var, ShadeArg<PRIMARY> arg)
+{
+    const int bounce = arg.bounce;
     __shared__ uint32_t sWaveE[2][TILE / 64], sWaveS[2][TILE / 64], sBaseE, sBaseS;
     enum { P_EXT_O, P_EXT_D, P_EXT_I, P_SH_A, P_SH_C, P_ROWS4 = NEE ? 5 : 3 };
     __shared__ float4 sPark4[P_ROWS4 * TILE + kShadeTableRows];
@@ -1548,7 +1576,8 @@
     auto fetch = [&](uint32_t t, TileIn& in) {
         const int j = (int)t * TILE + threadIdx.x;
         if (t < numTiles && j < n) {
-            in.hit = ldnt4(&q.hit[j]); in.meta = ldnt2(&q.meta[cur][j]); in.O = ldnt4(&q.O[cur][j]); in.D = ldnt4(&q.D[cur][j]); in.inten = ldnt4(&q.inten[cur][j]);
+            in.hit = ldnt4(&q.hit[j]);
+            if (!PRIMARY) { in.meta = ldnt2(&q.meta[cur][j]); in.O = ldnt4(&q.O[cur][j]); in.D = ldnt4(&q.D[cur][j]); in.inten = ldnt4(&q.inten[cur][j]); }
             in.seed = q.seeds[j];
         }
     };
@@ -1587,15 +1616,23 @@
         uint2 extMeta = make_uint2(0u, 0u);
         if (i < n) {
             const float4 hit = in.hit;
-            const uint2 meta = in.meta;
             SRay ray;
-            ray.O = in.O; ray.D = in.D; ray.inten = in.inten;
+            uint32_t seed = in.seed;
+            if (PRIMARY) {
+                ray.pixel = q.firstPixel + i; ray.bounces = 0; ray.inside = false; ray.lastSpec = true;
+                if constexpr (PRIMARY) primary_ray<REFB>(arg.gen.cam, ray.pixel % q.width, ray.pixel / q.width, q.width, q.height, arg.gen.aa, seed, ray.O, ray.D);
+                ray.inten = splat(1.0f);
+            } else {
+                const uint2 meta = in.meta;
+                ray.O = in.O; ray.D = in.D; ray.inten = in.inten;
+                ray.pixel = (int)meta.x; ray.bounces = (int)(meta.y & kMetaBounceMask);
+                ray.inside = (meta.y & kMetaInside) != 0; ray.lastSpec = (meta.y & kMetaLastSpec) != 0;
+            }
             ray.t = hit.x; ray.prim = __float_as_int(hit.y); ray.u = hit.z; ray.v = hit.w;
-            ray.pixel = (int)meta.x; ray.bounces = (int)(meta.y & kMetaBounceMask);
-            ray.inside = (meta.y & kMetaInside) != 0; ray.lastSpec = (meta.y & kMetaLastSpec) != 0;
             if (ray.prim == -1) {
                 float4 c = mul4(ray.inten, mk4(0.0784f, 0.0941f, 0.3215f, 0.0f));
                 q.accum[ray.pixel] = add4(q.accum[ray.pixel], c);
+                if (PRIMARY) q.seeds[i] = seed;
             } else {
                 ray.I = add4(ray.O, muls(ray.D, ray.t));
                 const float4 rec = sc.shadeRecs[ray.prim];
@@ -1605,7 +1642,6 @@
                 ray.N = (tag >> 28) == RT_PRIM_SPHERE ? prim_normal(sc.prims + ray.prim, ray.I)
                                                       : mk4(rec.x, rec.y, rec.z, (tag & 0x08000000u) ? -0.0f : 0.0f);
                 if (dot4(ray.N, neg4(ray.D)) < 0) ray.N = muls(ray.N, -1.0f);
-                uint32_t seed = in.seed;
                 float4 color = shade_hit<NEE, REFB>(sc, tab, var, ray, seed, ext, sh);
                 q.seeds[i] = seed;
                 color = firefly<REFB>(var.fireflies, color);
diff --git a/magr_ray_tracer_amd/csrc/trav_common.h b/magr_ray_tracer_amd/csrc/trav_common.h
--- a/magr_ray_tracer_amd/csrc/trav_common.h
+++ b/magr_ray_tracer_amd/csrc/trav_common.h
@@ -60,6 +60,7 @@
     bool xcdRaysSet = false; int xcdRays = 0;
     bool thinSet = false; int thin = 0;
     int connectBlocks = 0;
+    bool noFusePrimary = false;
 };
 
 static inline TravKnobs read_trav_knobs()
@@ -90,6 +91,7 @@
     if (const char* t = getenv("RT355_XCD_RAYS")) { k.xcdRays = std::max(0, atoi(t)); k.xcdRaysSet = true; }
     if (const char* t = getenv("RT355_THIN")) { k.thin = std::min(64, std::max(0, atoi(t))); k.thinSet = true; }
     if (const char* t = getenv("RT355_CONNECT_BLOCKS")) { const int d = atoi(t); if (d > 0) k.connectBlocks = d; }
+    if (const char* t = getenv("RT355_FUSE_PRIMARY")) k.noFusePrimary = atoi(t) == 0;
     return k;
 }
 
@@ -100,6 +102,7 @@
     PersistTune tune{}, tuneConnect{}, tune4{};
     bool topAuto = false;
     int tuneBlocks = 0, connectBlocks = 0;
+    bool fusePrimary = false;
 };
 
 static inline TravPlan plan_traversal(const TravFacts& f, const TravKnobs& k)
@@ -124,6 +127,7 @@
         else if (!fits) p.trav = TRAV_NESTED;
     }
     p.coherent = k.coherentSet ? k.coherent : 1;
+    p.fusePrimary = !k.noFusePrimary && ((p.trav == TRAV_BVH2 && f.extend_variant != 3 && f.extend_variant != 5) || p.trav == TRAV_BVH4);
 
     p.tune = PersistTune{ 112, 24, 6, 8, 0 }; p.tuneConnect = PersistTune{ 128, 32, 6, 16, 0 }; p.tune4 = PersistTune{ 64, 20, 6, 8, 0 };
     if (f.persist_blocks_per_cu > 0) {
diff --git a/magr_ray_tracer_amd/renderer.py b/magr_ray_tracer_amd/renderer.py
--- a/magr_ray_tracer_amd/renderer.py
+++ b/magr_ray_tracer_amd/renderer.py
@@ -424,6 +424,11 @@
         self._chk(self._lib.rt_shade_tables(self._h, C.byref(r), C.byref(s)))
         return int(r.value), bool(s.value)
 
+    def primary_fused(self):
+        f = C.c_int32(0)
+        self._chk(self._lib.rt_primary_fused(self._h, C.byref(f)))
+        return bool(f.value)
+
     @property
     def builtins(self):
         rc = self._lib.rt_builtins(self._h)
```
